# ZhishuaiGuo/DistributedAUC

Hardware: AMD Instinct MI355X
Metric: CoDA train imgs/sec + exact-AUC pos×neg pairs/sec at 1/2/4/8 MI355X (higher is better)
Workload: dtype bf16

## Files before the change

distributedauc_amd/_lib.py:

```python
from __future__ import annotations

import contextlib
import ctypes
import os
import re
from pathlib import Path

PKG_DIR = Path(__file__).resolve().parent
LIB_PATH = Path(os.environ.get("DAUC_LIB", PKG_DIR / "libdauc.so"))
HEADER = PKG_DIR.parent / "include" / "dauc.h"

DAUC_OK = 0
DAUC_EINVAL = -100000
LABEL_I8, LABEL_I32, LABEL_I64 = 1, 2, 3
DTYPE_F32, DTYPE_BF16 = 1, 2
MODE_REFERENCE, MODE_PAPER = 0, 1


class DaucError(RuntimeError):
    """A libdauc.so call returned a non-zero status."""


class GradSeg(ctypes.Structure):

    _fields_ = [("grad", ctypes.c_void_p), ("offset", ctypes.c_int64), ("numel", ctypes.c_int64)]


_vp = ctypes.c_void_p
_i64 = ctypes.c_int64
_int = ctypes.c_int
_f32 = ctypes.c_float
_sz = ctypes.c_size_t

SIGNATURES = {
    "dauc_version": (_int, []),
    "dauc_strerror": (ctypes.c_char_p, [_int]),
    "dauc_label_map_phat": (_int, [_vp, _i64, _i64, _vp, _vp, _vp, _vp, _vp]),
    "dauc_surrogate_workspace_size": (_sz, [_i64]),
    "dauc_surrogate_fwdbwd": (_int, [_vp, _i64, _vp, _int, _i64, _vp, _vp, _vp, _i64, _vp, _vp, _vp,
                                     _vp, _sz, _vp]),
    "dauc_class_sums": (_int, [_vp, _i64, _vp, _int, _i64, _vp, _int, _vp, _sz, _vp]),
    "dauc_surrogate_status": (_int, [_vp, _sz, _vp, _int, _vp]),
    "dauc_alpha_from_sums": (_int, [_vp, _vp, _vp]),
    "dauc_surrogate_logits_fwdbwd": (_int, [_vp, _int, _i64, _vp, _int, _i64, _vp, _vp, _vp, _i64, _vp, _vp,
                                            _vp, _vp, _vp, _sz, _vp]),
    "dauc_class_sums_logits": (_int, [_vp, _int, _i64, _vp, _int, _i64, _vp, _vp, _int, _vp, _sz, _vp]),
    "dauc_pd_update": (_int, [_vp, _vp, _vp, ctypes.POINTER(GradSeg), _int, _vp, _vp, _vp, _f32, _f32,
                              _int, _vp]),
    "dauc_pd_update_dense": (_int, [_vp, _vp, _vp, _vp, _i64, _f32, _f32, _vp]),
    "dauc_coda_finalize": (_int, [_vp, _i64, _int, _vp, _vp, _vp]),
    "dauc_scale_div": (_int, [_vp, _i64, _f32, _vp]),
    "dauc_split_workspace_size": (_sz, [_i64]),
    "dauc_split_scores": (_int, [_vp, _vp, _int, _i64, _vp, _vp, _vp, _vp, _sz, _vp]),
    "dauc_pair_count": (_int, [_vp, _i64, _vp, _i64, _vp, _vp]),
    "dauc_sort_workspace_size": (_sz, [_i64]),
    "dauc_auc_counts_sorted": (_int, [_vp, _i64, _vp, _i64, _vp, _vp, _sz, _vp]),
    "dauc_auc_counts_sorted_labeled": (_int, [_vp, _i64, _vp, _vp, _int, _i64, _i64, _vp, _vp, _vp, _sz, _vp]),
    "dauc_compact_workspace_size": (_sz, [_i64]),
    "dauc_auc_eval_workspace_size": (_sz, [_i64]),
    "dauc_auc_eval_enqueue": (_int, [_vp, _vp, _int, _i64, _int, _int, _vp, _vp, _sz, _vp]),
    "dauc_auc_eval_counts": (_int, [_vp, _vp, _int, _i64, _vp, _vp, _vp, _sz, _vp]),
    "dauc_auc_eval_counts_part": (_int, [_vp, _vp, _int, _i64, _int, _int, _vp, _vp, _vp, _vp, _sz, _vp]),
    "dauc_auc_slot_bytes": (_sz, [_i64, _int]),
    "dauc_auc_eval_compact_part": (_int, [_vp, _vp, _int, _i64, _int, _int, _vp, _vp, _sz, _vp]),
    "dauc_auc_eval_query_part": (_int, [_vp, _vp, _int, _i64, _int, _int, _vp, _vp, _vp, _sz, _vp]),
    "dauc_auc_eval_query_part_sorted": (_int, [_vp, _vp, _int, _i64, _int, _int, _vp, _i64, _vp, _vp, _sz, _vp]),
    "dauc_compact_positives": (_int, [_vp, _vp, _int, _i64, _vp, _vp, _vp, _sz, _vp]),
    "dauc_sort_keys": (_int, [_vp, _i64, _vp, _vp, _sz, _vp]),
    "dauc_bn_workspace_size": (_sz, [_i64, _int]),
    "dauc_bn_act_forward": (_int, [_vp, _int, _i64, _int, _vp, _int, _vp, _vp, _vp, _vp, _f32, _f32, _vp, _vp, _vp,
                                   _vp, _vp, _sz, _vp]),
    "dauc_bn_act_backward": (_int, [_vp, _vp, _vp, _vp, _int, _i64, _int, _int, _vp, _vp, _vp, _vp, _vp, _vp, _vp,
                                    _vp, _sz, _vp]),
    "dauc_maxpool2d_forward": (_int, [_vp, _int, _i64, _int, _int, _int, _int, _int, _int, _vp, _vp, _int, _int,
                                      _vp]),
    "dauc_slab_sum": (_int, [_vp, _i64, _i64, _vp, _vp]),
    "dauc_conv3x3_wgrad_workspace_size": (_sz, [_i64, _int, _int, _int, _int]),
    "dauc_conv3x3_wgrad": (_int, [_vp, _vp, _int, _i64, _int, _int, _int, _int, _int, _int, _int, _vp, _vp, _sz,
                                  _vp]),
    "dauc_maxpool2d_backward": (_int, [_vp, _vp, _int, _i64, _int, _int, _int, _int, _int, _int, _int, _int, _vp,
                                       _vp]),
    "dauc_conv7x7s2_stem_forward": (_int, [_vp, _vp, _int, _i64, _int, _int, _int, _int, _vp, _vp]),
    "dauc_conv7x7s2_stem_wgrad_workspace_size": (_sz, [_i64, _int, _int]),
    "dauc_conv7x7s2_stem_wgrad": (_int, [_vp, _vp, _int, _i64, _int, _int, _int, _int, _vp, _vp, _sz, _vp]),
    "dauc_strided_pick": (_int, [_vp, _int, _i64, _int, _int, _int, _int, _vp, _vp]),
    "dauc_strided_add": (_int, [_vp, _int, _i64, _int, _int, _int, _int, _vp, _vp]),
    "dauc_broadcast_hw": (_int, [_vp, _int, _i64, _i64, _int, _vp, _vp]),
}

TUNING_SIGNATURES = {
    "dauc_surrogate_fwdbwd_variant": (_int, [_vp, _i64, _vp, _int, _i64, _vp, _vp, _vp, _i64, _vp, _vp, _vp,
                                             _vp, _sz, _int, _vp]),
    "dauc_pd_update_dense_variant": (_int, [_vp, _vp, _vp, _vp, _i64, _f32, _f32, _int, _vp]),
    "dauc_pair_count_variant": (_int, [_vp, _i64, _vp, _i64, _vp, _int, _vp]),
    "dauc_set_search_mode": (_int, [_int]),
    "dauc_set_direct_fault": (_int, [_int]),
    "dauc_set_index_form": (_int, [_int]),
    "dauc_probe_tr16": (_int, [_vp, _vp]),
    "dauc_set_wgrad_form": (_int, [_int]),
    "dauc_bn_launch_plan": (_int, [_i64, _int, _int, ctypes.POINTER(_i64)]),
    "dauc_conv3x3_wgrad_launch_plan": (_int, [_i64, _int, _int, _int, _int, _int, _int, _int, ctypes.POINTER(_i64)]),
}
BN_PLAN_WORDS = 12
WGRAD_PLAN_WORDS = 18
TUNING_LIB_PATH = Path(os.environ.get("DAUC_TUNING_LIB", PKG_DIR.parent / "tuning" / "libdauc_tuning.so"))

_lib = None
_tuning = None


@contextlib.contextmanager
def using(lib: ctypes.CDLL):
    global _lib
    prev = load()
    _lib = lib
    try:
        yield lib
    finally:
        _lib = prev


def header_functions(header: Path = HEADER) -> list[str]:
    text = re.sub(r"/\*.*?\*/", "", header.read_text(), flags=re.S)
    return sorted(set(re.findall(r"\b(dauc_[a-z0-9_]+)\s*\(", text)) - {"dauc_grad_seg"})


def load() -> ctypes.CDLL:
    global _lib
    if _lib is not None:
        return _lib
    if not LIB_PATH.exists():
        raise ImportError(
            f"{LIB_PATH} not found: the HIP library must be built first "
            "(python -c 'import __graft_entry__ as g; g.build()' or python distributedauc_amd/build.py). "
            "distributedauc_amd has no CPU fallback."
        )
    _lib = _attach(ctypes.CDLL(str(LIB_PATH)))
    return _lib


def _attach(lib: ctypes.CDLL) -> ctypes.CDLL:
    for name, (res, args) in SIGNATURES.items():
        fn = getattr(lib, name)
        fn.restype = res
        fn.argtypes = args
    for name, (res, args) in TUNING_SIGNATURES.items():
        if hasattr(lib, name):
            fn = getattr(lib, name)
            fn.restype = res
            fn.argtypes = args
    return lib


def tuning() -> ctypes.CDLL:
    global _tuning
    lib = load()
    if all(hasattr(lib, n) for n in TUNING_SIGNATURES):
        return lib
    if _tuning is None:
        if not TUNING_LIB_PATH.exists():
            raise ImportError(f"{TUNING_LIB_PATH} not found: build it with python distributedauc_amd/build.py")
        _tuning = _attach(ctypes.CDLL(str(TUNING_LIB_PATH)))
    return _tuning


def strerror(rc: int) -> str:
    return load().dauc_strerror(rc).decode()


def check(rc: int, what: str) -> None:
    if rc != DAUC_OK:
        raise DaucError(f"{what} failed: {strerror(rc)} (status {rc})")
```

distributedauc_amd/backbone.py:

```python
from __future__ import annotations

import weakref

import torch
import torch.nn as nn
import torch.nn.functional as F

__all__ = [
    "ResNet", "resnet18", "resnet34", "resnet50", "resnet101", "resnet152", "resnext50_32x4d",
    "resnext101_32x8d", "wide_resnet50_2", "wide_resnet101_2", "build_backbone",
]


def _bn_act(fused: bool, bn: nn.BatchNorm2d, x: torch.Tensor, relu: bool = True,
            residual: torch.Tensor | None = None) -> torch.Tensor:
    if fused and bn.training:
        from .fused_bn import bn_act

        return bn_act(x, bn, relu, residual)
    y = bn(x)
    if residual is not None:
        y = y + residual
    return F.relu(y, inplace=True) if relu else y


_shadow_live: list = []


class WeightShadow:

    def __init__(self, model: nn.Module, dgrad_fwd: bool = False, wgrad_hip: bool = False):
        flat = getattr(model, "_dauc_flat", None)
        if flat is None:
            raise RuntimeError("the weight shadow mirrors the FlatState buffer: build CoDA / FlatState first")
        self.src = flat.params
        self._model = weakref.ref(model)
        self.wgrad_hip = bool(wgrad_hip)
        dev = self.src.device
        convs = {id(m.weight): m for m in model.modules() if isinstance(m, nn.Conv2d)}
        idx, foff, vspec, fspec = [], 0, {}, {}
        for _, p, off, _n in flat.entries:
            m = convs.get(id(p))
            if m is None:
                continue
            vspec[id(p)] = (p.shape, p.stride(), off)
            if dgrad_fwd and _dgrad_as_fwd_ok(m):
                co, ci, k, _ = p.shape
                s0, s1, s2, s3 = p.stride()
                r = torch.arange(k)
                src = (off + torch.arange(co).view(1, co, 1, 1) * s0 + torch.arange(ci).view(ci, 1, 1, 1) * s1
                       + (k - 1 - r).view(1, 1, k, 1) * s2 + (k - 1 - r).view(1, 1, 1, k) * s3)
                idx.append(src.permute(0, 2, 3, 1).reshape(-1))
                fspec[id(p)] = ((ci, co, k, k), (k * k * co, 1, k * co, co), foff)
                foff += p.numel()
        self.fidx = torch.cat(idx).to(device=dev, dtype=torch.int32) if idx else None
        self._sets = []
        for _ in range(2):
            buf = torch.empty(self.src.numel(), dtype=torch.bfloat16, device=dev)
            fbuf = torch.empty(foff, dtype=torch.bfloat16, device=dev) if foff else None
            views = {k: torch.as_strided(buf, sh, st, o) for k, (sh, st, o) in vspec.items()}
            flips = {k: torch.as_strided(fbuf, sh, st, o) for k, (sh, st, o) in fspec.items()}
            self._sets.append((buf, fbuf, views, flips))
        self._cur = 1
        self.buf, self.fbuf, self.views, self.flips = self._sets[0]

    def refresh(self, flips: bool = True) -> None:
        m = self._model()
        flat = getattr(m, "_dauc_flat", None) if m is not None else None
        if flat is None or flat.params is not self.src:
            raise RuntimeError("weight shadow is stale: the model's parameters moved to a new FlatState; call "
                               "model.set_weight_shadow(...) again after building it (CoDA does)")
        self._cur ^= 1
        self.buf, self.fbuf, self.views, self.flips = self._sets[self._cur]
        self.buf.copy_(self.src)
        if flips and self.fbuf is not None:
            torch.index_select(self.buf, 0, self.fidx, out=self.fbuf)

    def weight(self, p: torch.Tensor) -> torch.Tensor | None:
        return self.views.get(id(p))

    def flipped(self, p: torch.Tensor) -> torch.Tensor | None:
        return self.flips.get(id(p))


def _dgrad_as_fwd_ok(m: nn.Conv2d) -> bool:
    k = m.kernel_size
    return (k[0] == k[1] and k[0] % 2 == 1 and k[0] > 1 and m.stride == (1, 1) and m.dilation == (1, 1)
            and m.groups == 1 and not isinstance(m.padding, str) and tuple(m.padding) == (k[0] // 2, k[0] // 2)
            and m.padding_mode == "zeros")


def shadow_weight(p: torch.Tensor, dtype: torch.dtype) -> torch.Tensor | None:
    if not _shadow_live or dtype != torch.bfloat16:
        return None
    return _shadow_live[-1].weight(p)


class _ShadowConv(torch.autograd.Function):

    @staticmethod
    def forward(ctx, x, weight, wb, wf, stride, padding, dilation, groups, wgrad_hip=False):
        ctx.stem = False
        if wgrad_hip:
            from . import ops

            ctx.stem = ops.stem_conv_supported(x, wb, stride, padding, dilation, groups)
        if ctx.stem:
            y = ops.stem_conv_forward(x, wb)
        else:
            with torch.autocast("cuda", enabled=False):
                y = F.conv2d(x, wb, None, stride, padding, dilation, groups)
        ctx.save_for_backward(x, wb, wf)
        ctx.conf = (list(stride), list(padding), list(dilation), groups)
        ctx.wgrad_hip = bool(wgrad_hip)
        return y

    @staticmethod
    def backward(ctx, gy):
        x, wb, wf = ctx.saved_tensors
        stride, padding, dilation, groups = ctx.conf
        nx, nw = bool(ctx.needs_input_grad[0]), bool(ctx.needs_input_grad[1])
        dx = dw = None
        if nw and ctx.stem and gy.dtype == torch.bfloat16:
            from . import ops

            dw = ops.stem_conv_wgrad(x, gy.contiguous(memory_format=torch.channels_last))
        elif nw and ctx.wgrad_hip and wb.shape[2:] == (3, 3):
            from . import ops

            gyc = gy.contiguous(memory_format=torch.channels_last)
            if ops.conv3x3_wgrad_supported(x, gyc, stride, padding, dilation, groups):
                dw = ops.conv3x3_wgrad(x, gyc, stride[0])
        mw = nw and dw is None
        if wf is not None and nx:
            dx = F.conv2d(gy.contiguous(memory_format=torch.channels_last), wf, None, 1, padding, 1, 1)
            if mw:
                dw = torch.ops.aten.convolution_backward(gy, x, wb, None, stride, padding, dilation, False, [0, 0],
                                                         groups, [False, True, False])[1].float()
        elif nx or mw:
            dx, dwb, _ = torch.ops.aten.convolution_backward(gy, x, wb, None, stride, padding, dilation, False,
                                                              [0, 0], groups, [nx, mw, False])
            if mw:
                dw = dwb.float()
        return dx, dw, None, None, None, None, None, None, None


def _cw(conv: nn.Conv2d, x: torch.Tensor) -> torch.Tensor:
    wb = shadow_weight(conv.weight, torch.bfloat16) if x.is_cuda else None
    if (wb is None or conv.bias is not None or conv.padding_mode != "zeros" or isinstance(conv.padding, str)
            or not torch.is_autocast_enabled("cuda")):
        return conv(x)
    if x.dtype == torch.float32:
        x = x.to(torch.bfloat16)
    if x.dtype != torch.bfloat16:
        return conv(x)
    sh = _shadow_live[-1]
    wf = sh.flipped(conv.weight) if torch.is_grad_enabled() else None
    return _ShadowConv.apply(x, conv.weight, wb, wf, conv.stride, conv.padding, conv.dilation, conv.groups,
                             sh.wgrad_hip)


class _GlobalAvgPoolCL(torch.autograd.Function):

    @staticmethod
    def forward(ctx, x):
        ctx.shape = x.shape
        return F.adaptive_avg_pool2d(x, 1)

    @staticmethod
    def backward(ctx, g):
        N, C, H, W = ctx.shape
        gs = g / (H * W)
        if gs.is_cuda and gs.dtype == torch.bfloat16 and C % 8 == 0:
            from . import ops

            return ops.broadcast_hw(gs, H, W)
        out = torch.empty((N, C, H, W), dtype=gs.dtype, device=gs.device, memory_format=torch.channels_last)
        out.copy_(gs.expand(N, C, H, W))
        return out


def _global_pool(pool: nn.Module, x: torch.Tensor) -> torch.Tensor:
    if (x.is_cuda and x.dim() == 4 and x.is_contiguous(memory_format=torch.channels_last)
            and isinstance(pool, nn.AdaptiveAvgPool2d) and pool.output_size in (1, (1, 1)) and torch.is_grad_enabled()):
        return _GlobalAvgPoolCL.apply(x)
    return pool(x)


def _c1(gemm: bool, conv: nn.Conv2d, x: torch.Tensor) -> torch.Tensor:
    if gemm:
        from .conv1x1 import conv1x1

        return conv1x1(conv, x)
    return conv(x)


def _conv(cin: int, cout: int, k: int, stride: int = 1, groups: int = 1) -> nn.Conv2d:
    return nn.Conv2d(cin, cout, kernel_size=k, stride=stride, padding=k // 2, groups=groups, bias=False)


class BasicBlock(nn.Module):
    expansion = 1

    def __init__(self, cin, planes, stride=1, downsample=None, groups=1, base_width=64):
        super().__init__()
        if groups != 1 or base_width != 64:
            raise ValueError("BasicBlock supports groups=1, base_width=64 only")
        self.conv1 = _conv(cin, planes, 3, stride)
        self.bn1 = nn.BatchNorm2d(planes)
        self.conv2 = _conv(planes, planes, 3)
        self.bn2 = nn.BatchNorm2d(planes)
        self.relu = nn.ReLU(inplace=True)
        self.downsample = downsample
        self.fused_bn = False
        self.gemm_conv1x1 = False

    def forward(self, x):
        f = self.fused_bn
        skip = x if self.downsample is None else _bn_act(f, self.downsample[1], _c1(self.gemm_conv1x1,
                                                                                  self.downsample[0], x),
                                                         relu=False)
        y = _bn_act(f, self.bn1, _cw(self.conv1, x))
        return _bn_act(f, self.bn2, _cw(self.conv2, y), residual=skip)


class Bottleneck(nn.Module):

    expansion = 4

    def __init__(self, cin, planes, stride=1, downsample=None, groups=1, base_width=64):
        super().__init__()
        width = int(planes * (base_width / 64.0)) * groups
        self.conv1 = _conv(cin, width, 1)
        self.bn1 = nn.BatchNorm2d(width)
        self.conv2 = _conv(width, width, 3, stride, groups)
        self.bn2 = nn.BatchNorm2d(width)
        self.conv3 = _conv(width, planes * self.expansion, 1)
        self.bn3 = nn.BatchNorm2d(planes * self.expansion)
        self.relu = nn.ReLU(inplace=True)
        self.downsample = downsample
        self.fused_bn = False
        self.gemm_conv1x1 = False

    def forward(self, x):
        f, g = self.fused_bn, self.gemm_conv1x1
        down = None if self.downsample is None else self.downsample[0]
        if g and x.is_cuda:
            from .conv1x1 import conv1x1_skip

            h, skip = conv1x1_skip(self.conv1, x, down, skip_grad_owned=f and self.training)
        else:
            h, skip = _c1(g, self.conv1, x), (x if down is None else _c1(g, down, x))
        if down is not None:
            skip = _bn_act(f, self.downsample[1], skip, relu=False)
        y = _bn_act(f, self.bn1, h)
        y = _bn_act(f, self.bn2, _cw(self.conv2, y))
        return _bn_act(f, self.bn3, _c1(g, self.conv3, y), residual=skip)


class ResNet(nn.Module):

    def __init__(self, block, layers, num_classes: int = 2, groups: int = 1, width_per_group: int = 64,
                 zero_init_residual: bool = False, head: str = "softmax"):
        super().__init__()
        if head not in ("softmax", "logits"):
            raise ValueError("head must be 'softmax' or 'logits'")
        self.groups = groups
        self.base_width = width_per_group
        self.inplanes = 64
        self.conv1 = nn.Conv2d(3, 64, kernel_size=7, stride=2, padding=3, bias=False)
        self.bn1 = nn.BatchNorm2d(64)
        self.relu = nn.ReLU(inplace=True)
        self.maxpool = nn.MaxPool2d(kernel_size=3, stride=2, padding=1)
        self.layer1 = self._stage(block, 64, layers[0], 1)
        self.layer2 = self._stage(block, 128, layers[1], 2)
        self.layer3 = self._stage(block, 256, layers[2], 2)
        self.layer4 = self._stage(block, 512, layers[3], 2)
        self.avgpool = nn.AdaptiveAvgPool2d((1, 1))
        self.fc = nn.Linear(512 * block.expansion, num_classes)
        self.softmax = nn.Softmax(dim=1) if head == "softmax" else nn.Identity()
        for m in self.modules():
            if isinstance(m, nn.Conv2d):
                nn.init.kaiming_normal_(m.weight, mode="fan_out", nonlinearity="relu")
            elif isinstance(m, nn.BatchNorm2d):
                nn.init.ones_(m.weight)
                nn.init.zeros_(m.bias)
        if zero_init_residual:
            for m in self.modules():
                if isinstance(m, Bottleneck):
                    nn.init.zeros_(m.bn3.weight)
                elif isinstance(m, BasicBlock):
                    nn.init.zeros_(m.bn2.weight)

    def _stage(self, block, planes, blocks, stride):
        down = None
        cout = planes * block.expansion
        if stride != 1 or self.inplanes != cout:
            down = nn.Sequential(_conv(self.inplanes, cout, 1, stride), nn.BatchNorm2d(cout))
        mods = [block(self.inplanes, planes, stride, down, self.groups, self.base_width)]
        self.inplanes = cout
        mods += [block(cout, planes, 1, None, self.groups, self.base_width) for _ in range(1, blocks)]
        return nn.Sequential(*mods)

    fused_bn = False
    _counted_bns: list = []
    _wshadow: WeightShadow | None = None

    def set_weight_shadow(self, enabled: bool = True, dgrad_fwd: bool = True, wgrad_hip: bool = True) -> "ResNet":
        self._wshadow = WeightShadow(self, dgrad_fwd=dgrad_fwd, wgrad_hip=wgrad_hip) if enabled else None
        return self

    def set_fused_bn(self, enabled: bool = True) -> "ResNet":
        self.fused_bn = bool(enabled)
        self._counted_bns = []
        for m in self.modules():
            if isinstance(m, (BasicBlock, Bottleneck)):
                m.fused_bn = self.fused_bn
            if isinstance(m, nn.BatchNorm2d):
                batched = self.fused_bn and m.track_running_stats and m.momentum is not None
                m._dauc_counted = batched
                if batched:
                    self._counted_bns.append(m)
        return self

    def set_gemm_conv1x1(self, enabled: bool = True) -> "ResNet":
        for m in self.modules():
            if isinstance(m, (BasicBlock, Bottleneck)):
                m.gemm_conv1x1 = bool(enabled)
        return self

    def features(self, x):
        if self.fused_bn and self.training and x.is_cuda and self._counted_bns:
            torch._foreach_add_([m.num_batches_tracked for m in self._counted_bns], 1)
        live = (self._wshadow is not None and x.is_cuda and torch.is_autocast_enabled("cuda")
                and torch.get_autocast_dtype("cuda") == torch.bfloat16)
        if live:
            self._wshadow.refresh(flips=torch.is_grad_enabled())
            _shadow_live.append(self._wshadow)
        try:
            x = _bn_act(self.fused_bn, self.bn1, _cw(self.conv1, x))
            if self.fused_bn and x.is_cuda:
                from .pool import max_pool2d

                x = max_pool2d(x, self.maxpool)
            else:
                x = self.maxpool(x)
            x = self.layer4(self.layer3(self.layer2(self.layer1(x))))
        finally:
            if live:
                _shadow_live.pop()
        return torch.flatten(_global_pool(self.avgpool, x), 1)

    def forward(self, x):
        return self.softmax(self.fc(self.features(x)))


_SPECS = {
    "resnet18": (BasicBlock, [2, 2, 2, 2], {}),
    "resnet34": (BasicBlock, [3, 4, 6, 3], {}),
    "resnet50": (Bottleneck, [3, 4, 6, 3], {}),
    "resnet101": (Bottleneck, [3, 4, 23, 3], {}),
    "resnet152": (Bottleneck, [3, 8, 36, 3], {}),
    "resnext50_32x4d": (Bottleneck, [3, 4, 6, 3], {"groups": 32, "width_per_group": 4}),
    "resnext101_32x8d": (Bottleneck, [3, 4, 23, 3], {"groups": 32, "width_per_group": 8}),
    "wide_resnet50_2": (Bottleneck, [3, 4, 6, 3], {"width_per_group": 128}),
    "wide_resnet101_2": (Bottleneck, [3, 4, 23, 3], {"width_per_group": 128}),
}


def build_backbone(arch: str, pretrained: bool | str = False, **kwargs) -> ResNet:
    block, layers, extra = _SPECS[arch]
    model = ResNet(block, layers, **{**extra, **kwargs})
    if pretrained:
        if pretrained is True:
            raise RuntimeError("pretrained weights need a local state_dict path (no network in this build)")
        sd = torch.load(pretrained, map_location="cpu", weights_only=True)
        sd = {k: v for k, v in sd.items() if not k.startswith("fc.")}
        model.load_state_dict(sd, strict=False)
    return model


def _factory(name):
    def make(pretrained=False, progress=True, **kwargs):
        return build_backbone(name, pretrained, **kwargs)

    make.__name__ = name
    make.__doc__ = f"{name} with a 2-way softmax head (resnet.py factory of the same name)."
    return make


resnet18 = _factory("resnet18")
resnet34 = _factory("resnet34")
resnet50 = _factory("resnet50")
resnet101 = _factory("resnet101")
resnet152 = _factory("resnet152")
resnext50_32x4d = _factory("resnext50_32x4d")
resnext101_32x8d = _factory("resnext101_32x8d")
wide_resnet50_2 = _factory("wide_resnet50_2")
wide_resnet101_2 = _factory("wide_resnet101_2")
```

distributedauc_amd/conv1x1.py:

```python
from __future__ import annotations

import contextlib
import os

import torch
import torch.nn as nn
import torch.nn.functional as F

from . import _lib
from .ops import _ptr, _stream, check, strided_add_, strided_pick

__all__ = ["conv1x1", "conv1x1_skip", "Conv1x1Function", "Conv1x1SkipFunction", "plans", "dump_plans"]

plans: dict = {}

_DOWNSAMPLE_BWD = os.environ.get("DAUC_DOWNSAMPLE_BWD", "gemm")
PLANS_FILE = os.environ.get("DAUC_CONV1X1_PLANS", os.path.join(os.path.dirname(__file__), "conv1x1_plans.json"))


def _plan_key(key) -> str:
    M, cin, cout, dtype, direction = key
    return f"{M},{cin},{cout},{str(dtype).replace('torch.', '')},{direction}"


def _arch() -> str:
    return torch.cuda.get_device_properties(torch.cuda.current_device()).gcnArchName.split(":")[0]


def _load_plans() -> None:
    if not PLANS_FILE or not os.path.exists(PLANS_FILE):
        return
    import json

    dtypes = {"bfloat16": torch.bfloat16, "float16": torch.float16, "float32": torch.float32}
    with open(PLANS_FILE) as f:
        doc = json.load(f)
    if doc.get("arch") and torch.cuda.is_available() and doc["arch"] != _arch():
        return
    for k, eng in doc.get("plans", {}).items():
        M, cin, cout, dt, direction = k.split(",")
        plans.setdefault((int(M), int(cin), int(cout), dtypes[dt], direction), eng)


def dump_plans(path: str) -> None:
    import json

    with open(path, "w") as f:
        json.dump({"device": torch.cuda.get_device_name(0) if torch.cuda.is_available() else None,
                   "arch": _arch() if torch.cuda.is_available() else None,
                   "plans": {_plan_key(k): v for k, v in sorted(plans.items(), key=lambda kv: _plan_key(kv[0]))}},
                  f, indent=1)



def _timed(fn, reps=3):
    torch.cuda.synchronize()
    best = float("inf")
    for _ in range(reps):
        a, b = torch.cuda.Event(enable_timing=True), torch.cuda.Event(enable_timing=True)
        a.record()
        fn()
        b.record()
        b.synchronize()
        best = min(best, a.elapsed_time(b))
    return best


_FORCE = os.environ.get("DAUC_CONV1X1", "auto")
_loaded: list = []
_fixed: list = []


@contextlib.contextmanager
def fixed_engine(name: str = "gemm"):
    _fixed.append(name)
    try:
        yield
    finally:
        _fixed.pop()


def _choose(key, candidates: dict):
    if _fixed:
        eng = next((n for n in candidates if n.startswith(_fixed[-1])), None)
        if eng == "gemm8" and "gemm32" in candidates:
            eng = "gemm32"
        if eng is not None:
            return eng
    if not _loaded:
        _load_plans()
        _loaded.append(True)
    eng = plans.get(key) if _FORCE == "auto" else None
    if eng is None and _FORCE != "auto":
        eng = next((n for n in candidates if n.startswith(_FORCE)), None)
        if eng == "gemm8" and "gemm32" in candidates:
            eng = "gemm32"
        if eng is not None:
            plans[key] = eng
    if eng is None:
        times = {name: _timed(fn) for name, fn in candidates.items()}
        eng = min(times, key=times.get)
        plans[key] = eng
    return eng


def _wgrad_gemm(g2, x2, slabs):
    M, cout = g2.shape
    cin = x2.shape[1]
    if slabs == 1:
        return torch.mm(g2.t(), x2, out_dtype=torch.float32)
    part = torch.bmm(g2.view(slabs, M // slabs, cout).transpose(1, 2), x2.view(slabs, M // slabs, cin),
                     out_dtype=torch.float32)
    if (cout * cin) % 4:
        return part.sum(0)
    out = torch.empty((cout, cin), dtype=torch.float32, device=part.device)
    check(_lib.load().dauc_slab_sum(_ptr(part), slabs, cout * cin, _ptr(out), _stream(part.device)),
          "dauc_slab_sum")
    return out


def _low(weight, dtype):
    from .backbone import shadow_weight

    wb = shadow_weight(weight, dtype)
    return wb.detach() if wb is not None else weight.detach().to(dtype)


def _fwd(x, weight):
    N, cin, H, W = x.shape
    cout = weight.shape[0]
    M = N * H * W
    wc = _low(weight, x.dtype).reshape(cout, cin)
    x2 = x.permute(0, 2, 3, 1).reshape(M, cin)
    with torch.autocast("cuda", enabled=False):
        key = (M, cin, cout, x.dtype, "fwd")
        eng = _choose(key, {"gemm": lambda: torch.mm(x2, wc.t()),
                            "conv": lambda: F.conv2d(x, wc.view(cout, cin, 1, 1))})
        if eng == "gemm":
            y = torch.mm(x2, wc.t()).view(N, H, W, cout).permute(0, 3, 1, 2)
        else:
            y = F.conv2d(x, wc.view(cout, cin, 1, 1)).contiguous(memory_format=torch.channels_last)
    return y, wc


def _prep_grad(gy, x, cout):
    N, cin, H, W = x.shape
    gy = gy.to(x.dtype).contiguous(memory_format=torch.channels_last)
    return gy, gy.permute(0, 2, 3, 1).reshape(N * H * W, cout)


def _conv_dgrad(gy, x, wc):
    cout, cin = wc.shape
    return torch.ops.aten.convolution_backward(gy, x, wc.view(cout, cin, 1, 1), None, [1, 1], [0, 0], [1, 1],
                                               False, [0, 0], 1, [True, False, False])[0]


def _fconv_dgrad(gy, wc):
    cout, cin = wc.shape
    return F.conv2d(gy, wc.t().contiguous().view(cin, cout, 1, 1)).contiguous(memory_format=torch.channels_last)


def _dgrad(gy, g2, x, wc):
    N, cin, H, W = x.shape
    cout = wc.shape[0]
    M = N * H * W
    with torch.autocast("cuda", enabled=False):
        eng = _choose((M, cin, cout, x.dtype, "dgrad"),
                      {"gemm": lambda: torch.mm(g2, wc), "conv": lambda: _conv_dgrad(gy, x, wc),
                       "fconv": lambda: _fconv_dgrad(gy, wc)})
        if eng == "gemm":
            return torch.mm(g2, wc).view(N, H, W, cin).permute(0, 3, 1, 2)
        if eng == "fconv":
            return _fconv_dgrad(gy, wc)
        return _conv_dgrad(gy, x, wc).contiguous(memory_format=torch.channels_last)


def _dgrad_acc(base, gy, g2, x, wc):
    N, cin, H, W = x.shape
    cout = wc.shape[0]
    M = N * H * W
    b2 = base.permute(0, 2, 3, 1).reshape(M, cin)
    with torch.autocast("cuda", enabled=False):
        key = (M, cin, cout, x.dtype, "dgrad_acc")
        if not _loaded:
            _load_plans()
            _loaded.append(True)
        eng = None if _fixed else plans.get(key)
        if eng is None and _fixed:
            eng = _choose(key, {"gemm": None, "conv": None, "fconv": None})
        elif eng is None:
            scratch = base.clone(memory_format=torch.channels_last)
            s2 = scratch.permute(0, 2, 3, 1).reshape(M, cin)
            eng = _choose(key, {"gemm": lambda: s2.addmm_(g2, wc),
                                "conv": lambda: scratch.add_(_conv_dgrad(gy, x, wc)),
                                "fconv": lambda: scratch.add_(_fconv_dgrad(gy, wc))})
            del scratch, s2
        if eng == "gemm":
            b2.addmm_(g2, wc)
        elif eng == "fconv":
            base.add_(_fconv_dgrad(gy, wc))
        else:
            base.add_(_conv_dgrad(gy, x, wc))
    return base


def _wgrad(gy, g2, x, wc, wdtype):
    N, cin, H, W = x.shape
    cout = wc.shape[0]
    M = N * H * W
    x2 = x.permute(0, 2, 3, 1).reshape(M, cin)
    with torch.autocast("cuda", enabled=False):
        def conv_w():
            return torch.ops.aten.convolution_backward(gy, x, wc.view(cout, cin, 1, 1), None, [1, 1], [0, 0], [1, 1],
                                                       False, [0, 0], 1, [False, True, False])[1]

        cands = {"conv": conv_w}
        for s in (8, 32, 128):
            if M % s == 0 and M // s >= 64:
                cands[f"gemm{s}"] = (lambda s=s: _wgrad_gemm(g2, x2, s))
        eng = _choose((M, cin, cout, x.dtype, "wgrad"), cands)
        if eng == "conv":
            dw = conv_w().reshape(cout, cin).to(wdtype)
        else:
            dw = _wgrad_gemm(g2, x2, int(eng[4:])).to(wdtype)
    return dw.view(cout, cin, 1, 1)


def _cl_ok(t: torch.Tensor) -> bool:
    return (t.is_cuda and t.dtype == torch.bfloat16 and t.dim() == 4 and t.shape[1] % 8 == 0
            and t.is_contiguous(memory_format=torch.channels_last) and t.data_ptr() % 16 == 0)


def _pick(x: torch.Tensor, s: int) -> torch.Tensor:
    if _cl_ok(x):
        return strided_pick(x, s)
    return x[:, :, ::s, ::s].contiguous(memory_format=torch.channels_last)


def _add_strided(dx: torch.Tensor, src: torch.Tensor, s: int) -> None:
    if _cl_ok(dx) and _cl_ok(src):
        strided_add_(dx, src, s)
    else:
        dx[:, :, ::s, ::s].add_(src)


class Conv1x1Function(torch.autograd.Function):
    @staticmethod
    def forward(ctx, x, weight):
        y, wc = _fwd(x, weight)
        ctx.save_for_backward(x, wc)
        ctx.wdtype = weight.dtype
        return y

    @staticmethod
    def backward(ctx, gy):
        x, wc = ctx.saved_tensors
        gy, g2 = _prep_grad(gy, x, wc.shape[0])
        dx = _dgrad(gy, g2, x, wc) if ctx.needs_input_grad[0] else None
        dw = _wgrad(gy, g2, x, wc, ctx.wdtype) if ctx.needs_input_grad[1] else None
        return dx, dw


class Conv1x1SkipFunction(torch.autograd.Function):

    @staticmethod
    def forward(ctx, x, w1, wd, skip_grad_owned, down_stride=1):
        y1, wc1 = _fwd(x, w1)
        ctx.down_stride = int(down_stride)
        if wd is None:
            skip, wcd = x, None
        elif down_stride == 1:
            skip, wcd = _fwd(x, wd)
        else:
            wcd = _low(wd, x.dtype).reshape(wd.shape[0], wd.shape[1])
            with torch.autocast("cuda", enabled=False):
                skip = F.conv2d(x, wcd.view(*wd.shape), stride=down_stride).contiguous(
                    memory_format=torch.channels_last)
        ctx.save_for_backward(x, wc1, wcd)
        ctx.wdtypes = (w1.dtype, None if wd is None else wd.dtype)
        ctx.skip_grad_owned = bool(skip_grad_owned)
        return y1, skip

    @staticmethod
    def backward(ctx, g1, gs):
        x, wc1, wcd = ctx.saved_tensors
        dx = dw1 = dwd = None
        gy1 = g21 = gyd = g2d = None
        if g1 is not None:
            gy1, g21 = _prep_grad(g1, x, wc1.shape[0])
        strided = wcd is not None and ctx.down_stride != 1
        s = ctx.down_stride
        xd = x
        dx_down = dwd_s = None
        if gs is not None and strided and _DOWNSAMPLE_BWD == "miopen":
            gsd = gs.to(x.dtype).contiguous(memory_format=torch.channels_last)
            cout, cin = wcd.shape
            with torch.autocast("cuda", enabled=False):
                dx_down, dwd_s, _ = torch.ops.aten.convolution_backward(
                    gsd, x, wcd.view(cout, cin, 1, 1), None, [s, s], [0, 0], [1, 1], False, [0, 0], 1,
                    [bool(ctx.needs_input_grad[0]), bool(ctx.needs_input_grad[2]), False])
        elif gs is not None and wcd is not None:
            if strided:
                xd = _pick(x, s)
            gyd, g2d = _prep_grad(gs, xd, wcd.shape[0])
        if ctx.needs_input_grad[0]:
            if gs is None:
                base = None
            elif wcd is None:
                base = gs.to(x.dtype).contiguous(memory_format=torch.channels_last)
                if base is gs and not ctx.skip_grad_owned:
                    base = base.clone(memory_format=torch.channels_last)
            elif strided:
                base = None if dx_down is None else dx_down.contiguous(memory_format=torch.channels_last)
            else:
                base = _dgrad(gyd, g2d, x, wcd)
            if g1 is None:
                dx = base
            elif base is None:
                dx = _dgrad(gy1, g21, x, wc1)
            else:
                dx = _dgrad_acc(base, gy1, g21, x, wc1)
            if strided and gs is not None and dx_down is None:
                if dx is None:
                    dx = torch.zeros_like(x, memory_format=torch.channels_last)
                _add_strided(dx, _dgrad(gyd, g2d, xd, wcd), s)
        if ctx.needs_input_grad[1] and g1 is not None:
            dw1 = _wgrad(gy1, g21, x, wc1, ctx.wdtypes[0])
        if wcd is not None and ctx.needs_input_grad[2] and gs is not None:
            if dwd_s is not None:
                dwd = dwd_s.to(ctx.wdtypes[1]).view(wcd.shape[0], wcd.shape[1], 1, 1)
            else:
                dwd = _wgrad(gyd, g2d, xd, wcd, ctx.wdtypes[1])
        return dx, dw1, dwd, None, None


def conv1x1(conv: nn.Conv2d, x: torch.Tensor) -> torch.Tensor:
    if (conv.kernel_size != (1, 1) or conv.stride != (1, 1) or conv.groups != 1 or conv.bias is not None
            or conv.padding != (0, 0) or x.device.type != "cuda"
            or not x.is_contiguous(memory_format=torch.channels_last)):
        return conv(x)
    if torch.is_autocast_enabled("cuda") and x.dtype == torch.float32:
        x = x.to(torch.get_autocast_dtype("cuda"))
    return Conv1x1Function.apply(x, conv.weight)


def _gemm_ok(conv: nn.Conv2d | None, x: torch.Tensor, any_stride: bool = False) -> bool:
    return conv is None or (conv.kernel_size == (1, 1) and conv.groups == 1 and conv.bias is None
                            and conv.padding == (0, 0) and conv.dilation == (1, 1)
                            and (conv.stride == (1, 1) or (any_stride and conv.stride[0] == conv.stride[1])))


def conv1x1_skip(conv: nn.Conv2d, x: torch.Tensor, down: nn.Conv2d | None = None, skip_grad_owned: bool = False):
    if (x.device.type != "cuda" or not x.is_contiguous(memory_format=torch.channels_last)
            or not _gemm_ok(conv, x) or not _gemm_ok(down, x, any_stride=True)):
        return conv1x1(conv, x), (x if down is None else conv1x1(down, x))
    if torch.is_autocast_enabled("cuda") and x.dtype == torch.float32:
        x = x.to(torch.get_autocast_dtype("cuda"))
    return Conv1x1SkipFunction.apply(x, conv.weight, None if down is None else down.weight, skip_grad_owned,
                                     1 if down is None else down.stride[0])
```

distributedauc_amd/csrc/bn_act.hip:

```cpp

#include <hip/hip_bf16.h>

#include <initializer_list>
#include <type_traits>

#include "dauc_internal.h"
#ifdef DAUC_TUNING
#include "dauc_tuning.h"
#endif

namespace dauc {
namespace {

constexpr int kBnThreads = 256;
constexpr int kDefaultPartThreads = 512;
constexpr int kMaxRowBlocks = 2048;
constexpr int kFinThreads = 1024;
constexpr int kFinSubsets = kFinThreads / 16;

constexpr int kRowBlockTarget = 256;
static_assert(kRowBlockTarget >= 1 && kRowBlockTarget <= kMaxRowBlocks, "partial rows fit the workspace");
constexpr int kUnroll = 8;
constexpr int kFwdUnroll = kUnroll;
constexpr int kBwdUnroll = kUnroll / 2;
constexpr int kFinUnroll = 4;
constexpr int kApplyVecs = 4;
constexpr int64_t kApplyBlockVecs = int64_t(kApplyVecs) * kBnThreads;

template <typename T>
struct VecT;
template <>
struct VecT<__hip_bfloat16> {
    static constexpr int N = 8;
};
template <>
struct VecT<float> {
    static constexpr int N = 4;
};

template <typename T>
using RawT = typename std::conditional<sizeof(T) == 2, uint4, f32x4>::type;

template <typename T>
__device__ __forceinline__ RawT<T> load_raw(const T* p) {
    return *reinterpret_cast<const RawT<T>*>(p);
}

__device__ __forceinline__ void cvt(const uint4& u, float (&v)[8]) {
    const unsigned w[4] = {u.x, u.y, u.z, u.w};
#pragma unroll
    for (int i = 0; i < 4; ++i) {
        v[2 * i] = __uint_as_float(w[i] << 16);
        v[2 * i + 1] = __uint_as_float(w[i] & 0xffff0000u);
    }
}

__device__ __forceinline__ void cvt(const f32x4& u, float (&v)[4]) {
#pragma unroll
    for (int i = 0; i < 4; ++i) v[i] = u[i];
}

template <typename T, int N>
__device__ __forceinline__ void load_vec(const T* p, float (&v)[N]) {
    cvt(load_raw(p), v);
}

__device__ __forceinline__ unsigned bf16_bits(float f) {
    const unsigned b = __float_as_uint(f);
    if ((b & 0x7fffffffu) > 0x7f800000u) return (b >> 16) | 0x40u;
    return (b + 0x7fffu + ((b >> 16) & 1u)) >> 16;
}

__device__ __forceinline__ void store_vec(__hip_bfloat16* p, const float (&v)[8]) {
    uint4 u;
    u.x = bf16_bits(v[0]) | (bf16_bits(v[1]) << 16);
    u.y = bf16_bits(v[2]) | (bf16_bits(v[3]) << 16);
    u.z = bf16_bits(v[4]) | (bf16_bits(v[5]) << 16);
    u.w = bf16_bits(v[6]) | (bf16_bits(v[7]) << 16);
    *reinterpret_cast<uint4*>(p) = u;
}

__device__ __forceinline__ void store_vec(float* p, const float (&v)[4]) {
    f32x4 u;
#pragma unroll
    for (int i = 0; i < 4; ++i) u[i] = v[i];
    *reinterpret_cast<f32x4*>(p) = u;
}

__device__ __forceinline__ unsigned store_vec_mask(__hip_bfloat16* p, const float (&v)[8]) {
    unsigned b[8], m = 0u;
#pragma unroll
    for (int i = 0; i < 8; ++i) {
        b[i] = bf16_bits(v[i]);
        m |= unsigned(b[i] - 1u < 0x7f80u) << i;
    }
    uint4 u;
    u.x = b[0] | (b[1] << 16);
    u.y = b[2] | (b[3] << 16);
    u.z = b[4] | (b[5] << 16);
    u.w = b[6] | (b[7] << 16);
    *reinterpret_cast<uint4*>(p) = u;
    return m;
}

__device__ __forceinline__ unsigned store_vec_mask(float* p, const float (&v)[4]) {
    unsigned m = 0u;
#pragma unroll
    for (int i = 0; i < 4; ++i) m |= unsigned(__float_as_uint(v[i]) - 1u < 0x7f800000u) << i;
    store_vec(p, v);
    return m;
}

struct Geometry {
    int N;
    int CT;
    int TPR;
    int RPB;
    int ctiles;
    int nrb;
    int64_t rows;
};

int make_geometry(int64_t M, int C, int elem_bytes, Geometry& g, int threads = kBnThreads) {
    g.N = 16 / elem_bytes;
    if (M <= 0 || C <= 0 || C % g.N != 0) return DAUC_EINVAL;
    const int CV = C / g.N;
    g.TPR = CV <= kBnThreads ? CV : kBnThreads;
    if (kBnThreads % g.TPR != 0 || CV % g.TPR != 0) return DAUC_EINVAL;
    g.CT = g.TPR * g.N;
    g.ctiles = C / g.CT;
    g.RPB = threads / g.TPR;
    int64_t target = (kRowBlockTarget + g.ctiles - 1) / g.ctiles;
    const int64_t passes = (M + g.RPB - 1) / g.RPB;
    if (target > passes) target = passes;
    if (target < 1) target = 1;
    int64_t rows = (M + target - 1) / target;
    rows = (rows + g.RPB - 1) / g.RPB * g.RPB;
    g.rows = rows;
    g.nrb = static_cast<int>((M + rows - 1) / rows);
    return DAUC_OK;
}

template <typename T, bool STATS, bool RELU, int TH, bool MASK = false>
__global__ __launch_bounds__(TH) void bn_partial_kernel(
    const T* __restrict__ x, const T* __restrict__ dy, const T* __restrict__ y, T* __restrict__ dz, int64_t M,
    int C, int CT, int64_t rows_per_block, const float* __restrict__ center, float* __restrict__ partials,
    const unsigned char* __restrict__ mask) {
    constexpr int N = VecT<T>::N;
    __shared__ float red[2 * TH * N];
    const int TPR = CT / N;
    const int RPB = TH / TPR;
    const int cl = (threadIdx.x % TPR) * N;
    const int c0 = blockIdx.y * CT + cl;
    const int r0 = threadIdx.x / TPR;
    const int64_t rs = int64_t(blockIdx.x) * rows_per_block;
    const int64_t re = (rs + rows_per_block < M) ? rs + rows_per_block : M;
    constexpr int NP = STATS ? 3 : 2;

    float k[N], s1[N], s2[N];
    if (STATS) load_vec(x + rs * C + c0, k);
#pragma unroll
    for (int i = 0; i < N; ++i) {
        if (!STATS) k[i] = center[c0 + i];
        s1[i] = 0.f;
        s2[i] = 0.f;
    }
    auto visit = [&](int64_t r) {
        const int64_t off = r * C + c0;
        float xv[N];
        load_vec(x + off, xv);
        if (STATS) {
#pragma unroll
            for (int i = 0; i < N; ++i) {
                const float d = xv[i] - k[i];
                s1[i] += d;
                s2[i] += d * d;
            }
        } else {
            float gv[N];
            load_vec(dy + off, gv);
            if (RELU && MASK) {
                const unsigned m = mask[off / N];
#pragma unroll
                for (int i = 0; i < N; ++i) gv[i] = (m >> i) & 1u ? gv[i] : 0.f;
            } else if (RELU) {
                float yv[N];
                load_vec(y + off, yv);
#pragma unroll
                for (int i = 0; i < N; ++i) gv[i] = yv[i] > 0.f ? gv[i] : 0.f;
            }
            if (dz) store_vec(dz + off, gv);
#pragma unroll
            for (int i = 0; i < N; ++i) {
                s1[i] += gv[i];
                s2[i] += gv[i] * (xv[i] - k[i]);
            }
        }
    };
    constexpr int U = STATS ? kFwdUnroll : kBwdUnroll;
    int64_t r = rs + r0;
    const int64_t step = int64_t(RPB) * U;
    for (; r + step - RPB < re; r += step) {
        RawT<T> xr[U], gr[U], yr[U];
        unsigned mr[U];
#pragma unroll
        for (int u = 0; u < U; ++u) {
            const int64_t off = (r + int64_t(u) * RPB) * C + c0;
            xr[u] = load_raw(x + off);
            if (!STATS) gr[u] = load_raw(dy + off);
            if (!STATS && RELU && MASK) mr[u] = mask[off / N];
            else if (!STATS && RELU) yr[u] = load_raw(y + off);
        }
#pragma unroll
        for (int u = 0; u < U; ++u) {
            float xv[N];
            cvt(xr[u], xv);
            if (STATS) {
#pragma unroll
                for (int i = 0; i < N; ++i) {
                    const float d = xv[i] - k[i];
                    s1[i] += d;
                    s2[i] += d * d;
                }
            } else {
                float gv[N];
                cvt(gr[u], gv);
                if (RELU && MASK) {
#pragma unroll
                    for (int i = 0; i < N; ++i) gv[i] = (mr[u] >> i) & 1u ? gv[i] : 0.f;
                } else if (RELU) {
                    float yv[N];
                    cvt(yr[u], yv);
#pragma unroll
                    for (int i = 0; i < N; ++i) gv[i] = yv[i] > 0.f ? gv[i] : 0.f;
                }
                if (dz) store_vec(dz + (r + int64_t(u) * RPB) * C + c0, gv);
#pragma unroll
                for (int i = 0; i < N; ++i) {
                    s1[i] += gv[i];
                    s2[i] += gv[i] * (xv[i] - k[i]);
                }
            }
        }
    }
    for (; r < re; r += RPB) visit(r);

    float* r1 = red;
    float* r2 = red + TH * N;
#pragma unroll
    for (int i = 0; i < N; ++i) {
        r1[r0 * CT + cl + i] = s1[i];
        r2[r0 * CT + cl + i] = s2[i];
    }
    __syncthreads();
    for (int j = threadIdx.x; j < 2 * CT; j += TH) {
        const int stat = j / CT, c = j % CT;
        const float* src = stat ? r2 : r1;
        float acc = 0.f;
        for (int q = 0; q < RPB; ++q) acc += src[q * CT + c];
        partials[(int64_t(blockIdx.x) * NP + stat) * C + blockIdx.y * CT + c] = acc;
    }
    if (STATS && r0 == 0) {
#pragma unroll
        for (int i = 0; i < N; ++i) partials[(int64_t(blockIdx.x) * NP + 2) * C + c0 + i] = k[i];
    }
}

template <bool STATS>
__device__ __forceinline__ void sum_partials(const float* __restrict__ partials, int nrb, int64_t M, int64_t rows,
                                             int C, int cbase, double (*red)[kFinSubsets][64], double& t1,
                                             double& t2) {
    constexpr int NP = STATS ? 3 : 2;
    constexpr int FU = kFinUnroll;
    const int cq = threadIdx.x % 16, j = threadIdx.x / 16;
    const int c = cbase + cq * 4;
    double a1[4] = {0, 0, 0, 0}, a2[4] = {0, 0, 0, 0};
    auto fold = [&](int rb, const f32x4& p1, const f32x4& p2, const f32x4& pk) {
        if (STATS) {
            const int64_t r0 = int64_t(rb) * rows;
            const double nb = double((M - r0) < rows ? (M - r0) : rows);
#pragma unroll
            for (int i = 0; i < 4; ++i) {
                const double k = pk[i], s1 = p1[i];
                a1[i] += s1 + nb * k;
                a2[i] += double(p2[i]) + 2.0 * k * s1 + nb * k * k;
            }
        } else {
#pragma unroll
            for (int i = 0; i < 4; ++i) {
                a1[i] += p1[i];
                a2[i] += p2[i];
            }
        }
    };
    auto ld = [&](int rb, int q) {
        return *reinterpret_cast<const f32x4*>(partials + (int64_t(rb) * NP + q) * C + c);
    };
    if (c < C) {
        int rb = j;
        for (; rb + (FU - 1) * kFinSubsets < nrb; rb += FU * kFinSubsets) {
            f32x4 p1[FU], p2[FU], pk[FU];
#pragma unroll
            for (int u = 0; u < FU; ++u) {
                p1[u] = ld(rb + u * kFinSubsets, 0);
                p2[u] = ld(rb + u * kFinSubsets, 1);
                if (STATS) pk[u] = ld(rb + u * kFinSubsets, 2);
            }
#pragma unroll
            for (int u = 0; u < FU; ++u) fold(rb + u * kFinSubsets, p1[u], p2[u], pk[u]);
        }
        for (; rb < nrb; rb += kFinSubsets) {
            const f32x4 p1 = ld(rb, 0), p2 = ld(rb, 1);
            f32x4 pk;
            if (STATS) pk = ld(rb, 2);
            fold(rb, p1, p2, pk);
        }
    }
#pragma unroll
    for (int i = 0; i < 4; ++i) {
        red[0][j][cq * 4 + i] = a1[i];
        red[1][j][cq * 4 + i] = a2[i];
    }
    __syncthreads();
#pragma unroll
    for (int s = kFinSubsets / 2; s >= 1; s >>= 1) {
        if (j < s) {
#pragma unroll
            for (int i = 0; i < 4; ++i) {
                red[0][j][cq * 4 + i] += red[0][j + s][cq * 4 + i];
                red[1][j][cq * 4 + i] += red[1][j + s][cq * 4 + i];
            }
        }
        __syncthreads();
    }
    t1 = 0.0;
    t2 = 0.0;
    if (threadIdx.x < 64) {
        t1 = red[0][0][threadIdx.x];
        t2 = red[1][0][threadIdx.x];
    }
}

__global__ __launch_bounds__(kFinThreads) void bn_fwd_finalize_kernel(
    const float* __restrict__ partials, int nrb, int64_t rows, int64_t M, int C, const float* __restrict__ gamma,
    const float* __restrict__ beta, float* __restrict__ running_mean, float* __restrict__ running_var,
    float momentum, float eps, float* __restrict__ save_mean, float* __restrict__ save_invstd,
    float* __restrict__ scale, float* __restrict__ beta_out, float* __restrict__ mean_out) {
    __shared__ double red[2][kFinSubsets][64];
    double sx, sxx;
    sum_partials<true>(partials, nrb, M, rows, C, blockIdx.x * 64, red, sx, sxx);
    const int c = blockIdx.x * 64 + threadIdx.x;
    if (threadIdx.x >= 64 || c >= C) return;
    const double mean = sx / double(M);
    double var = sxx / double(M) - mean * mean;
    if (var < 0.0) var = 0.0;
    const double invstd = 1.0 / sqrt(var + double(eps));
    save_mean[c] = static_cast<float>(mean);
    save_invstd[c] = static_cast<float>(invstd);
    const double g = gamma ? gamma[c] : 1.0, b = beta ? beta[c] : 0.0;
    scale[c] = static_cast<float>(g * invstd);
    beta_out[c] = static_cast<float>(b);
    mean_out[c] = static_cast<float>(mean);
    if (running_mean) {
        const double unbiased = M > 1 ? var * double(M) / double(M - 1) : var;
        running_mean[c] = static_cast<float>((1.0 - momentum) * running_mean[c] + momentum * mean);
        running_var[c] = static_cast<float>((1.0 - momentum) * running_var[c] + momentum * unbiased);
    }
}

__global__ __launch_bounds__(kFinThreads) void bn_bwd_finalize_kernel(
    const float* __restrict__ partials, int nrb, int64_t M, int C, const float* __restrict__ gamma,
    const float* __restrict__ save_mean, const float* __restrict__ save_invstd, float* __restrict__ dgamma,
    float* __restrict__ dbeta, float* __restrict__ ca, float* __restrict__ cb, float* __restrict__ cc,
    float* __restrict__ cm) {
    __shared__ double red[2][kFinSubsets][64];
    double sg, sgx;
    sum_partials<false>(partials, nrb, M, 0, C, blockIdx.x * 64, red, sg, sgx);
    const int c = blockIdx.x * 64 + threadIdx.x;
    if (threadIdx.x >= 64 || c >= C) return;
    const double inv = save_invstd[c], mean = save_mean[c];
    const double g = gamma ? gamma[c] : 1.0;
    if (dgamma) dgamma[c] = static_cast<float>(sgx * inv);
    if (dbeta) dbeta[c] = static_cast<float>(sg);
    const double a = g * inv;
    const double b = -g * inv * inv * inv * sgx / double(M);
    ca[c] = static_cast<float>(a);
    cb[c] = static_cast<float>(b);
    cc[c] = static_cast<float>(-a * sg / double(M));
    cm[c] = save_mean[c];
}

template <typename T, bool BWD, int GMODE, bool RELU, bool RES, bool HOIST, bool MASK = false>
__global__ __launch_bounds__(kBnThreads) void bn_elementwise_kernel(
    const T* __restrict__ x, const T* __restrict__ g_in, const T* __restrict__ aux, T* __restrict__ out,
    int64_t nvec, int CV, const float* __restrict__ p0, const float* __restrict__ p1, const float* __restrict__ p2,
    const float* __restrict__ p3, unsigned char* __restrict__ mask) {
    constexpr int N = VecT<T>::N;
    auto body = [&](int64_t v, const float* P0, const float* P1, const float* P2, const float* P3) {
        const int64_t off = v * N;
        float xv[N];
        load_vec(x + off, xv);
        float o[N];
        if (!BWD) {
            float rv[N];
            if (RES) load_vec(aux + off, rv);
#pragma unroll
            for (int i = 0; i < N; ++i) {
                float t = (xv[i] - P3[i]) * P0[i] + P1[i];
                if (RES) t += rv[i];
                o[i] = (RELU && t < 0.f) ? 0.f : t;
            }
        } else {
            float gv[N];
            load_vec(g_in + off, gv);
            if (GMODE == 1 && MASK) {
                const unsigned m = mask[v];
#pragma unroll
                for (int i = 0; i < N; ++i) gv[i] = (m >> i) & 1u ? gv[i] : 0.f;
            } else if (GMODE == 1) {
                float yv[N];
                load_vec(aux + off, yv);
#pragma unroll
                for (int i = 0; i < N; ++i) gv[i] = yv[i] > 0.f ? gv[i] : 0.f;
            }
#pragma unroll
            for (int i = 0; i < N; ++i) o[i] = P0[i] * gv[i] + P1[i] * (xv[i] - P3[i]) + P2[i];
        }
        if constexpr (!BWD && RELU && MASK)
            mask[v] = static_cast<unsigned char>(store_vec_mask(out + off, o));
        else
            store_vec(out + off, o);
    };
    auto params = [&](int cv, float (&q0)[N], float (&q1)[N], float (&q2)[N], float (&q3)[N]) {
#pragma unroll
        for (int i = 0; i < N; ++i) {
            q0[i] = p0[cv * N + i];
            q1[i] = p1[cv * N + i];
            q2[i] = BWD ? p2[cv * N + i] : 0.f;
            q3[i] = p3[cv * N + i];
        }
    };
    const int64_t base = int64_t(blockIdx.x) * kApplyVecs * kBnThreads + threadIdx.x;
    float q0[N], q1[N], q2[N], q3[N];
    if (HOIST) params(threadIdx.x % CV, q0, q1, q2, q3);
    if (int64_t(blockIdx.x + 1) * kApplyVecs * kBnThreads <= nvec) {
#pragma unroll
        for (int u = 0; u < kApplyVecs; ++u) {
            const int64_t v = base + int64_t(u) * kBnThreads;
            if (!HOIST) params(static_cast<int>(v % CV), q0, q1, q2, q3);
            body(v, q0, q1, q2, q3);
        }
    } else {
        for (int u = 0; u < kApplyVecs; ++u) {
            const int64_t v = base + int64_t(u) * kBnThreads;
            if (v >= nvec) break;
            if (!HOIST) params(static_cast<int>(v % CV), q0, q1, q2, q3);
            body(v, q0, q1, q2, q3);
        }
    }
}

struct BnWs {
    float* partials;
    float* c0;
    float* c1;
    float* c2;
    float* c3;
};

size_t ws_bytes_for(int C) {
    return (size_t(kMaxRowBlocks) * 3 + 4) * size_t(C) * sizeof(float) + 256;
}

BnWs carve(void* ws, int C) {
    char* p = static_cast<char*>(ws);
    BnWs w;
    w.partials = reinterpret_cast<float*>(p);
    w.c0 = w.partials + size_t(kMaxRowBlocks) * 3 * C;
    w.c1 = w.c0 + C;
    w.c2 = w.c1 + C;
    w.c3 = w.c2 + C;
    return w;
}

bool aligned16p(const void* p) { return (reinterpret_cast<uintptr_t>(p) & 15u) == 0; }

int64_t apply_blocks(int64_t nvec) { return (nvec + kApplyBlockVecs - 1) / kApplyBlockVecs; }
bool apply_hoists(int CV) { return kBnThreads % CV == 0; }

template <typename T, bool BWD, int GMODE, bool RELU, bool RES, bool MASK = false>
int launch_elementwise(const T* x, const T* g_in, const T* aux, T* out, int64_t M, int C, const float* p0,
                       const float* p1, const float* p2, const float* p3, hipStream_t st,
                       unsigned char* mask = nullptr) {
    constexpr int N = VecT<T>::N;
    const int CV = C / N;
    const int64_t nvec = M * CV;
    const int64_t grid = apply_blocks(nvec);
    if (grid > 0x7fffffffLL) return DAUC_EINVAL;
    if (apply_hoists(CV))
        hipLaunchKernelGGL((bn_elementwise_kernel<T, BWD, GMODE, RELU, RES, true, MASK>), dim3(unsigned(grid)),
                           dim3(kBnThreads), 0, st, x, g_in, aux, out, nvec, CV, p0, p1, p2, p3, mask);
    else
        hipLaunchKernelGGL((bn_elementwise_kernel<T, BWD, GMODE, RELU, RES, false, MASK>), dim3(unsigned(grid)),
                           dim3(kBnThreads), 0, st, x, g_in, aux, out, nvec, CV, p0, p1, p2, p3, mask);
    return launch_status();
}

template <typename T, bool STATS, bool RELU, bool MASK = false>
void launch_partial(int th, const Geometry& g, const T* x, const T* dy, const T* y, T* dz, int64_t M, int C,
                    const float* center, float* partials, hipStream_t st, const unsigned char* mask = nullptr) {
    const dim3 grid(g.nrb, g.ctiles);
    if (th == 1024)
        hipLaunchKernelGGL((bn_partial_kernel<T, STATS, RELU, 1024, MASK>), grid, dim3(1024), 0, st, x, dy, y, dz, M,
                           C, g.CT, g.rows, center, partials, mask);
    else if (th == 512)
        hipLaunchKernelGGL((bn_partial_kernel<T, STATS, RELU, 512, MASK>), grid, dim3(512), 0, st, x, dy, y, dz, M,
                           C, g.CT, g.rows, center, partials, mask);
    else
        hipLaunchKernelGGL((bn_partial_kernel<T, STATS, RELU, 256, MASK>), grid, dim3(256), 0, st, x, dy, y, dz, M,
                           C, g.CT, g.rows, center, partials, mask);
}

template <typename T>
int bn_forward_t(const T* x, int64_t M, int C, const T* res, int relu, const float* gamma, const float* beta,
                 float* running_mean, float* running_var, float momentum, float eps, T* y, unsigned char* mask,
                 float* save_mean, float* save_invstd, void* ws, size_t ws_bytes, hipStream_t st) {
    Geometry g;
    const int th = kDefaultPartThreads;
    if (make_geometry(M, C, sizeof(T), g, th) != DAUC_OK) return DAUC_EINVAL;
    if (ws == nullptr || ws_bytes < ws_bytes_for(C) || !aligned16p(ws)) return DAUC_EINVAL;
    if ((running_mean == nullptr) != (running_var == nullptr)) return DAUC_EINVAL;
    const BnWs w = carve(ws, C);
    launch_partial<T, true, false>(th, g, x, nullptr, nullptr, nullptr, M, C, nullptr, w.partials, st);
    hipLaunchKernelGGL(bn_fwd_finalize_kernel, dim3((C + 63) / 64), dim3(kFinThreads), 0, st, w.partials, g.nrb,
                       g.rows, M, C, gamma, beta, running_mean, running_var, momentum, eps, save_mean, save_invstd, w.c0, w.c1, w.c3);
    int rc = launch_status();
    if (rc != DAUC_OK) return rc;
    if (relu && mask && res)
        return launch_elementwise<T, false, 0, true, true, true>(x, nullptr, res, y, M, C, w.c0, w.c1, nullptr, w.c3, st,
                                                                mask);
    if (relu && mask)
        return launch_elementwise<T, false, 0, true, false, true>(x, nullptr, nullptr, y, M, C, w.c0, w.c1, nullptr,
                                                                 w.c3, st, mask);
    if (relu && res)
        return launch_elementwise<T, false, 0, true, true>(x, nullptr, res, y, M, C, w.c0, w.c1, nullptr, w.c3, st);
    if (relu) return launch_elementwise<T, false, 0, true, false>(x, nullptr, nullptr, y, M, C, w.c0, w.c1, nullptr, w.c3, st);
    if (res) return launch_elementwise<T, false, 0, false, true>(x, nullptr, res, y, M, C, w.c0, w.c1, nullptr, w.c3, st);
    return launch_elementwise<T, false, 0, false, false>(x, nullptr, nullptr, y, M, C, w.c0, w.c1, nullptr, w.c3, st);
}

template <typename T>
int bn_backward_t(const T* dy, const T* y, const unsigned char* mask, const T* x, int64_t M, int C, int relu,
                  const float* gamma, const float* save_mean, const float* save_invstd, T* dres, T* dx, float* dgamma,
                  float* dbeta, void* ws, size_t ws_bytes, hipStream_t st) {
    Geometry g;
    const int th = kDefaultPartThreads;
    if (make_geometry(M, C, sizeof(T), g, th) != DAUC_OK) return DAUC_EINVAL;
    if (ws == nullptr || ws_bytes < ws_bytes_for(C) || !aligned16p(ws)) return DAUC_EINVAL;
    if (relu && y == nullptr && mask == nullptr) return DAUC_EINVAL;
    const BnWs w = carve(ws, C);
    if (relu && mask)
        launch_partial<T, false, true, true>(th, g, x, dy, nullptr, dres, M, C, save_mean, w.partials, st, mask);
    else if (relu)
        launch_partial<T, false, true>(th, g, x, dy, y, dres, M, C, save_mean, w.partials, st);
    else
        launch_partial<T, false, false>(th, g, x, dy, nullptr, dres, M, C, save_mean, w.partials, st);
    hipLaunchKernelGGL(bn_bwd_finalize_kernel, dim3((C + 63) / 64), dim3(kFinThreads), 0, st, w.partials, g.nrb, M, C,
                       gamma, save_mean, save_invstd, dgamma, dbeta, w.c0, w.c1, w.c2, w.c3);
    int rc = launch_status();
    if (rc != DAUC_OK) return rc;
    if (dres)
        return launch_elementwise<T, true, 2, false, false>(x, dres, nullptr, dx, M, C, w.c0, w.c1, w.c2, w.c3, st);
    if (relu && mask)
        return launch_elementwise<T, true, 1, false, false, true>(x, dy, nullptr, dx, M, C, w.c0, w.c1, w.c2, w.c3, st,
                                                                 const_cast<unsigned char*>(mask));
    if (relu) return launch_elementwise<T, true, 1, false, false>(x, dy, y, dx, M, C, w.c0, w.c1, w.c2, w.c3, st);
    return launch_elementwise<T, true, 0, false, false>(x, dy, nullptr, dx, M, C, w.c0, w.c1, w.c2, w.c3, st);
}

bool all_aligned(std::initializer_list<const void*> ps) {
    for (const void* p : ps)
        if (p != nullptr && !aligned16p(p)) return false;
    return true;
}

}
}

using namespace dauc;

extern "C" {

size_t dauc_bn_workspace_size(int64_t M, int C) {
    (void)M;
    return C > 0 ? ws_bytes_for(C) : 0;
}

int dauc_bn_act_forward(const void* x, int dtype, int64_t M, int C, const void* residual, int relu,
                        const float* gamma, const float* beta, float* running_mean, float* running_var,
                        float momentum, float eps, void* y, uint8_t* relu_mask, float* save_mean, float* save_invstd,
                        void* workspace, size_t workspace_bytes, dauc_stream_t stream) {
    if (x == nullptr || y == nullptr || save_mean == nullptr || save_invstd == nullptr) return DAUC_EINVAL;
    if (!all_aligned({x, residual, y})) return DAUC_EINVAL;
    if (relu_mask != nullptr && !relu) return DAUC_EINVAL;
    hipStream_t st = as_hip(stream);
    if (dtype == DAUC_DTYPE_BF16)
        return bn_forward_t(static_cast<const __hip_bfloat16*>(x), M, C, static_cast<const __hip_bfloat16*>(residual),
                            relu, gamma, beta, running_mean, running_var, momentum, eps,
                            static_cast<__hip_bfloat16*>(y), relu_mask, save_mean, save_invstd, workspace,
                            workspace_bytes, st);
    if (dtype == DAUC_DTYPE_F32)
        return bn_forward_t(static_cast<const float*>(x), M, C, static_cast<const float*>(residual), relu, gamma,
                            beta, running_mean, running_var, momentum, eps, static_cast<float*>(y), relu_mask,
                            save_mean, save_invstd, workspace, workspace_bytes, st);
    return DAUC_EINVAL;
}

int dauc_bn_act_backward(const void* dy, const void* y, const uint8_t* relu_mask, const void* x, int dtype, int64_t M,
                         int C, int relu, const float* gamma, const float* save_mean, const float* save_invstd,
                         void* dres, void* dx, float* dgamma, float* dbeta, void* workspace, size_t workspace_bytes,
                         dauc_stream_t stream) {
    if (dy == nullptr || x == nullptr || dx == nullptr || save_mean == nullptr || save_invstd == nullptr)
        return DAUC_EINVAL;
    if (!all_aligned({dy, y, x, dres, dx})) return DAUC_EINVAL;
    hipStream_t st = as_hip(stream);
    if (dtype == DAUC_DTYPE_BF16)
        return bn_backward_t(static_cast<const __hip_bfloat16*>(dy), static_cast<const __hip_bfloat16*>(y), relu_mask,
                             static_cast<const __hip_bfloat16*>(x), M, C, relu, gamma, save_mean, save_invstd,
                             static_cast<__hip_bfloat16*>(dres), static_cast<__hip_bfloat16*>(dx), dgamma, dbeta,
                             workspace, workspace_bytes, st);
    if (dtype == DAUC_DTYPE_F32)
        return bn_backward_t(static_cast<const float*>(dy), static_cast<const float*>(y), relu_mask,
                             static_cast<const float*>(x), M, C, relu, gamma, save_mean, save_invstd,
                             static_cast<float*>(dres), static_cast<float*>(dx), dgamma, dbeta, workspace,
                             workspace_bytes, st);
    return DAUC_EINVAL;
}

#ifdef DAUC_TUNING
int dauc_bn_launch_plan(int64_t M, int C, int dtype, int64_t out[DAUC_BN_PLAN_WORDS]) {
    if (out == nullptr || (dtype != DAUC_DTYPE_BF16 && dtype != DAUC_DTYPE_F32)) return DAUC_EINVAL;
    Geometry g;
    const int rc = make_geometry(M, C, dtype == DAUC_DTYPE_BF16 ? 2 : 4, g, kDefaultPartThreads);
    if (rc != DAUC_OK) return rc;
    const int CV = C / g.N;
    out[0] = g.TPR;
    out[1] = g.RPB;
    out[2] = g.ctiles;
    out[3] = g.nrb;
    out[4] = g.rows;
    out[5] = int64_t(g.RPB) * kFwdUnroll;
    out[6] = int64_t(g.RPB) * kBwdUnroll;
    out[7] = int64_t(kFinSubsets) * kFinUnroll;
    out[8] = kFinSubsets;
    out[9] = kApplyBlockVecs;
    out[10] = apply_blocks(M * CV);
    out[11] = apply_hoists(CV) ? 1 : 0;
    return DAUC_OK;
}
#endif

}
```

distributedauc_amd/csrc/dauc_internal.h:

```cpp
#pragma once

#include <hip/hip_runtime.h>
#include <stdint.h>

#include "../../include/dauc.h"

namespace dauc {

constexpr int kWave = 64;

typedef float f32x4 __attribute__((ext_vector_type(4)));

inline hipStream_t as_hip(dauc_stream_t s) { return reinterpret_cast<hipStream_t>(s); }

inline int launch_status() {
    hipError_t e = hipGetLastError();
    return e == hipSuccess ? DAUC_OK : -static_cast<int>(e);
}


__device__ __forceinline__ double wave_sum(double v) {
#pragma unroll
    for (int off = 32; off > 0; off >>= 1) v += __shfl_xor(v, off, kWave);
    return v;
}

__device__ __forceinline__ unsigned long long wave_sum(unsigned long long v) {
#pragma unroll
    for (int off = 32; off > 0; off >>= 1) v += __shfl_xor(v, off, kWave);
    return v;
}

template <int K>
__device__ __forceinline__ void block_sum(double (&v)[K], double* scratch) {
    const int lane = threadIdx.x & (kWave - 1);
    const int wid = threadIdx.x / kWave;
    const int nw = blockDim.x / kWave;
#pragma unroll
    for (int k = 0; k < K; ++k) v[k] = wave_sum(v[k]);
    if (lane == 0) {
#pragma unroll
        for (int k = 0; k < K; ++k) scratch[k * nw + wid] = v[k];
    }
    __syncthreads();
#pragma unroll
    for (int k = 0; k < K; ++k) {
        double s = 0.0;
        for (int w = 0; w < nw; ++w) s += scratch[k * nw + w];
        v[k] = s;
    }
    __syncthreads();
}

typedef __attribute__((address_space(1))) unsigned long long gu64;
typedef __attribute__((address_space(1))) unsigned gu32;

__device__ __forceinline__ void store_sc1(double* p, double v) {
    __hip_atomic_store((gu64*)p, static_cast<unsigned long long>(__double_as_longlong(v)), __ATOMIC_RELAXED,
                       __HIP_MEMORY_SCOPE_AGENT);
}

__device__ __forceinline__ double load_sc1(const double* p) {
    return __longlong_as_double(static_cast<long long>(
        __hip_atomic_load((gu64*)p, __ATOMIC_RELAXED, __HIP_MEMORY_SCOPE_AGENT)));
}

__device__ __forceinline__ bool arrive_last(unsigned* counter, unsigned nblocks, int* lds_flag) {
    if (threadIdx.x == 0) {
        asm volatile("s_waitcnt vmcnt(0)" ::: "memory");
        const unsigned t = __hip_atomic_fetch_add((gu32*)counter, 1u, __ATOMIC_RELAXED, __HIP_MEMORY_SCOPE_AGENT);
        const int last = (t == nblocks - 1);
        if (last) __hip_atomic_store((gu32*)counter, 0u, __ATOMIC_RELAXED, __HIP_MEMORY_SCOPE_AGENT);
        *lds_flag = last;
    }
    __syncthreads();
    __builtin_amdgcn_fence(__ATOMIC_ACQUIRE, "wavefront");
    return *lds_flag != 0;
}

inline bool label_dtype_ok(int label_dtype) {
    return label_dtype == DAUC_LABEL_I8 || label_dtype == DAUC_LABEL_I32 || label_dtype == DAUC_LABEL_I64;
}

template <typename F>
int with_labels(const void* labels, int label_dtype, F&& f) {
    switch (label_dtype) {
        case DAUC_LABEL_I8: return f(static_cast<const int8_t*>(labels));
        case DAUC_LABEL_I32: return f(static_cast<const int32_t*>(labels));
        case DAUC_LABEL_I64: return f(static_cast<const int64_t*>(labels));
        default: return DAUC_EINVAL;
    }
}

}
```

distributedauc_amd/fused_bn.py:

```python
from __future__ import annotations

import torch
import torch.nn as nn

from . import _lib
from .ops import _ptr, _stream, check, workspaces

__all__ = ["supported", "bn_act", "BnActFunction"]

_DTYPES = {torch.float32: 1, torch.bfloat16: 2}


def supported(x: torch.Tensor) -> bool:
    if x.dim() != 4 or x.device.type != "cuda" or x.dtype not in _DTYPES:
        return False
    if not x.is_contiguous(memory_format=torch.channels_last) or x.data_ptr() % 16:
        return False
    vec = 16 // x.element_size()
    C = x.shape[1]
    if C % vec:
        return False
    cv = C // vec
    tpr = min(cv, 256)
    return 256 % tpr == 0 and cv % tpr == 0


class BnActFunction(torch.autograd.Function):

    @staticmethod
    def forward(ctx, x, weight, bias, residual, running_mean, running_var, momentum, eps, relu):
        N, C, H, W = x.shape
        M = N * H * W
        dev = x.device
        L = _lib.load()
        y = torch.empty_like(x, memory_format=torch.channels_last)
        mask = torch.empty(M * C * x.element_size() // 16, dtype=torch.uint8, device=dev) if relu else None
        mean = torch.empty(C, dtype=torch.float32, device=dev)
        invstd = torch.empty(C, dtype=torch.float32, device=dev)
        ws = workspaces.get(dev, "bn", L.dauc_bn_workspace_size(M, C))
        if residual is not None:
            if residual.shape != x.shape or residual.dtype != x.dtype:
                raise ValueError("residual must match x in shape and dtype")
            residual = residual.contiguous(memory_format=torch.channels_last)
        check(L.dauc_bn_act_forward(_ptr(x), _DTYPES[x.dtype], M, C, _ptr(residual), int(relu), _ptr(weight),
                                    _ptr(bias), _ptr(running_mean), _ptr(running_var), float(momentum), float(eps),
                                    _ptr(y), _ptr(mask), _ptr(mean), _ptr(invstd), _ptr(ws), ws.numel(), _stream(dev)),
              "dauc_bn_act_forward")
        ctx.save_for_backward(x, mask, weight, mean, invstd)
        ctx.relu = bool(relu)
        ctx.has_residual = residual is not None
        ctx.has_bias = bias is not None
        return y

    @staticmethod
    def backward(ctx, dy):
        x, mask, weight, mean, invstd = ctx.saved_tensors
        N, C, H, W = x.shape
        M = N * H * W
        dev = x.device
        L = _lib.load()
        dy = dy.contiguous(memory_format=torch.channels_last)
        if dy.dtype != x.dtype:
            dy = dy.to(x.dtype)
        dx = torch.empty_like(x, memory_format=torch.channels_last)
        dres = torch.empty_like(x, memory_format=torch.channels_last) if ctx.has_residual else None
        dgamma = torch.empty(C, dtype=torch.float32, device=dev) if weight is not None else None
        dbeta = torch.empty(C, dtype=torch.float32, device=dev) if ctx.has_bias else None
        ws = workspaces.get(dev, "bn", L.dauc_bn_workspace_size(M, C))
        check(L.dauc_bn_act_backward(_ptr(dy), None, _ptr(mask), _ptr(x), _DTYPES[x.dtype], M, C, int(ctx.relu),
                                     _ptr(weight), _ptr(mean), _ptr(invstd), _ptr(dres), _ptr(dx), _ptr(dgamma),
                                     _ptr(dbeta), _ptr(ws), ws.numel(), _stream(dev)),
              "dauc_bn_act_backward")
        return dx, dgamma, dbeta, dres, None, None, None, None, None


def bn_act(x: torch.Tensor, bn: nn.BatchNorm2d, relu: bool = True,
           residual: torch.Tensor | None = None) -> torch.Tensor:
    if x.device.type != "cuda":
        raise RuntimeError("fused BN runs on the GPU only (libdauc.so); no CPU path")
    if not supported(x):
        raise ValueError(f"fused BN needs a channels-last bf16/fp32 tensor with a supported channel count, "
                         f"got {tuple(x.shape)} {x.dtype}")
    momentum = 0.0 if bn.momentum is None else bn.momentum
    rm, rv = (bn.running_mean, bn.running_var) if bn.track_running_stats else (None, None)
    if bn.track_running_stats and bn.num_batches_tracked is not None and not getattr(bn, "_dauc_counted", False):
        bn.num_batches_tracked.add_(1)
        if bn.momentum is None:
            momentum = 1.0 / float(bn.num_batches_tracked.item())
    return BnActFunction.apply(x, bn.weight, bn.bias, residual, rm, rv, momentum, bn.eps, relu)
```

include/dauc.h:

```cpp
#ifndef DAUC_H_
#define DAUC_H_

#include <stddef.h>
#include <stdint.h>

#ifdef __cplusplus
extern "C" {
#endif

typedef struct ihipStream_t* dauc_stream_t;

#define DAUC_OK 0
#define DAUC_EINVAL (-100000)

#define DAUC_LABEL_I8 1
#define DAUC_LABEL_I32 2
#define DAUC_LABEL_I64 3

#define DAUC_DTYPE_F32 1
#define DAUC_DTYPE_BF16 2

#define DAUC_MODE_REFERENCE 0
#define DAUC_MODE_PAPER 1


int dauc_version(void);

const char* dauc_strerror(int status);


int dauc_label_map_phat(const int64_t* labels, int64_t B, int64_t split_index, int8_t* y_out,
                        float* lcounts, const float* gcounts, float* p_hat, dauc_stream_t stream);


size_t dauc_surrogate_workspace_size(int64_t B);

int dauc_surrogate_fwdbwd(const float* h, int64_t h_stride, const void* y, int y_dtype, int64_t B,
                          const float* abalpha, const float* p_hat, float* dh, int64_t dh_stride,
                          double* out64, float* grad3, float* loss, void* workspace,
                          size_t workspace_bytes, dauc_stream_t stream);

int dauc_surrogate_status(void* workspace, size_t workspace_bytes, unsigned* status_out, int clear,
                          dauc_stream_t stream);

int dauc_class_sums(const float* h, int64_t h_stride, const void* y, int y_dtype, int64_t B,
                    double* sums4, int accumulate, void* workspace, size_t workspace_bytes,
                    dauc_stream_t stream);

int dauc_surrogate_logits_fwdbwd(const void* z, int z_dtype, int64_t ldz, const void* y, int y_dtype,
                                 int64_t B, const float* abalpha, const float* p_hat, void* dz, int64_t lddz,
                                 float* h_out, double* out64, float* grad3, float* loss, void* workspace,
                                 size_t workspace_bytes, dauc_stream_t stream);

int dauc_class_sums_logits(const void* z, int z_dtype, int64_t ldz, const void* y, int y_dtype, int64_t B,
                           float* h_out, double* sums4, int accumulate, void* workspace, size_t workspace_bytes,
                           dauc_stream_t stream);

int dauc_alpha_from_sums(const double* sums4, float* alpha, dauc_stream_t stream);


typedef struct dauc_grad_seg {
    const float* grad;
    int64_t offset;
    int64_t numel;
} dauc_grad_seg;

int dauc_pd_update(float* w, const float* w0, float* w_avg, const dauc_grad_seg* segs, int nseg,
                   float* scalars, const float* grad3, const float* anchor3, float lr,
                   float inv_gamma, int mode, dauc_stream_t stream);

int dauc_pd_update_dense(float* w, const float* g, const float* w0, float* w_avg, int64_t n,
                         float lr, float inv_gamma, dauc_stream_t stream);


int dauc_coda_finalize(float* flat, int64_t n_avg, int world, float* lcounts, float* gcounts,
                       dauc_stream_t stream);

int dauc_scale_div(float* x, int64_t n, float divisor, dauc_stream_t stream);


size_t dauc_split_workspace_size(int64_t n);

int dauc_split_scores(const float* scores, const void* labels, int label_dtype, int64_t n,
                      float* pos_out, float* neg_out, int64_t* stats, void* workspace,
                      size_t workspace_bytes, dauc_stream_t stream);

size_t dauc_compact_workspace_size(int64_t n);
int dauc_compact_positives(const float* scores, const void* labels, int label_dtype, int64_t n,
                           float* pos_out, int64_t* stats, void* workspace, size_t workspace_bytes,
                           dauc_stream_t stream);

int dauc_pair_count(const float* pos, int64_t P, const float* neg, int64_t N,
                    unsigned long long* wins_ties, dauc_stream_t stream);

size_t dauc_sort_workspace_size(int64_t n);

int dauc_auc_counts_sorted(const float* pos, int64_t P, const float* neg, int64_t N,
                           unsigned long long* wins_ties, void* workspace, size_t workspace_bytes,
                           dauc_stream_t stream);

int dauc_auc_counts_sorted_labeled(const float* pos, int64_t P, const float* scores, const void* labels,
                                   int label_dtype, int64_t begin, int64_t end, unsigned long long* wins_ties,
                                   unsigned long long* nonfinite, void* workspace, size_t workspace_bytes,
                                   dauc_stream_t stream);

size_t dauc_auc_eval_workspace_size(int64_t n);
int dauc_auc_eval_enqueue(const float* scores, const void* labels, int label_dtype, int64_t n, int part, int parts,
                          int64_t* part_out, void* workspace, size_t workspace_bytes, dauc_stream_t stream);

int dauc_auc_eval_counts(const float* scores, const void* labels, int label_dtype, int64_t n, int64_t* out,
                         int64_t* pinned, void* workspace, size_t workspace_bytes, dauc_stream_t stream);

int dauc_auc_eval_counts_part(const float* scores, const void* labels, int label_dtype, int64_t n, int part,
                              int parts, int64_t* out, int64_t* part_counts, int64_t* pinned, void* workspace,
                              size_t workspace_bytes, dauc_stream_t stream);

size_t dauc_auc_slot_bytes(int64_t n, int parts);
int dauc_auc_eval_compact_part(const float* scores, const void* labels, int label_dtype, int64_t n, int part,
                               int parts, void* slot, void* workspace, size_t workspace_bytes, dauc_stream_t stream);
int dauc_auc_eval_query_part(const float* scores, const void* labels, int label_dtype, int64_t n, int part, int parts,
                             const void* slots, int64_t* part_out, void* workspace, size_t workspace_bytes,
                             dauc_stream_t stream);
int dauc_auc_eval_query_part_sorted(const float* scores, const void* labels, int label_dtype, int64_t n, int part,
                                    int parts, const void* slots, int64_t P, int64_t* part_out, void* workspace,
                                    size_t workspace_bytes, dauc_stream_t stream);

int dauc_sort_keys(const float* scores, int64_t n, unsigned* keys_out, void* workspace,
                   size_t workspace_bytes, dauc_stream_t stream);


size_t dauc_bn_workspace_size(int64_t M, int C);
int dauc_bn_act_forward(const void* x, int dtype, int64_t M, int C, const void* residual, int relu,
                        const float* gamma, const float* beta, float* running_mean, float* running_var,
                        float momentum, float eps, void* y, uint8_t* relu_mask, float* save_mean, float* save_invstd,
                        void* workspace, size_t workspace_bytes, dauc_stream_t stream);

int dauc_bn_act_backward(const void* dy, const void* y, const uint8_t* relu_mask, const void* x, int dtype, int64_t M,
                         int C, int relu, const float* gamma, const float* save_mean, const float* save_invstd,
                         void* dres, void* dx, float* dgamma, float* dbeta, void* workspace, size_t workspace_bytes,
                         dauc_stream_t stream);


int dauc_maxpool2d_forward(const void* x, int dtype, int64_t N, int H, int W, int C, int kernel, int stride,
                           int pad, void* y, int8_t* argmax, int Ho, int Wo, dauc_stream_t stream);

int dauc_maxpool2d_backward(const void* dy, const int8_t* argmax, int dtype, int64_t N, int H, int W, int C,
                            int kernel, int stride, int pad, int Ho, int Wo, void* dx, dauc_stream_t stream);


int dauc_slab_sum(const float* part, int64_t S, int64_t n, float* out, dauc_stream_t stream);


size_t dauc_conv3x3_wgrad_workspace_size(int64_t N, int Ho, int Wo, int Ci, int Co);
int dauc_conv3x3_wgrad(const void* x, const void* dy, int dtype, int64_t N, int H, int W, int Ci, int Ho, int Wo,
                       int Co, int stride, float* dw, void* workspace, size_t workspace_bytes, dauc_stream_t stream);


int dauc_conv7x7s2_stem_forward(const void* x, const void* w, int dtype, int64_t N, int H, int W, int Ho, int Wo,
                                void* y, dauc_stream_t stream);
size_t dauc_conv7x7s2_stem_wgrad_workspace_size(int64_t N, int Ho, int Wo);
int dauc_conv7x7s2_stem_wgrad(const void* x, const void* dy, int dtype, int64_t N, int H, int W, int Ho, int Wo,
                              float* dw, void* workspace, size_t workspace_bytes, dauc_stream_t stream);


int dauc_strided_pick(const void* x, int dtype, int64_t N, int H, int W, int C, int stride, void* out,
                      dauc_stream_t stream);
int dauc_strided_add(void* dx, int dtype, int64_t N, int H, int W, int C, int stride, const void* src,
                     dauc_stream_t stream);
int dauc_broadcast_hw(const void* g, int dtype, int64_t N, int64_t HW, int C, void* out, dauc_stream_t stream);

#ifdef __cplusplus
}
#endif

#endif
```

include/dauc_tuning.h:

```cpp
#ifndef DAUC_TUNING_H
#define DAUC_TUNING_H

#include "dauc.h"

#ifdef __cplusplus
extern "C" {
#endif

int dauc_surrogate_fwdbwd_variant(const float* h, int64_t h_stride, const void* y, int y_dtype, int64_t B,
                                  const float* abalpha, const float* p_hat, float* dh, int64_t dh_stride,
                                  double* out64, float* grad3, float* loss, void* workspace,
                                  size_t workspace_bytes, int variant, dauc_stream_t stream);

int dauc_pd_update_dense_variant(float* w, const float* g, const float* w0, float* w_avg, int64_t n,
                                 float lr, float inv_gamma, int variant, dauc_stream_t stream);

int dauc_pair_count_variant(const float* pos, int64_t P, const float* neg, int64_t N,
                            unsigned long long* wins_ties, int variant, dauc_stream_t stream);

int dauc_set_search_mode(int mode);

int dauc_set_direct_fault(int mode);

int dauc_set_index_form(int form);

int dauc_probe_tr16(short* out, dauc_stream_t stream);

int dauc_set_wgrad_form(int form);

#define DAUC_BN_PLAN_WORDS 12
int dauc_bn_launch_plan(int64_t M, int C, int dtype, int64_t out[DAUC_BN_PLAN_WORDS]);

#define DAUC_WGRAD_PLAN_WORDS 18
int dauc_conv3x3_wgrad_launch_plan(int64_t N, int H, int W, int Ci, int Ho, int Wo, int Co, int stride,
                                   int64_t out[DAUC_WGRAD_PLAN_WORDS]);

#ifdef __cplusplus
}
#endif

#endif
```

Baseline: 11180.

## Fuse BN statistic partials into the 1x1 conv forward GEMM epilogue

Adds a HIP 1x1-conv forward kernel that emits per-row-block sum and sum-of-squares partials for the following BatchNorm in its epilogue. A new BN forward entry consumes these partials instead of rereading the conv output to compute statistics. Bottleneck blocks use this path for conv1, the stride-1 downsample and conv3 when fused BN and the GEMM conv are on, with an autotune choice against the library GEMM per shape. It saves one full read of each activation tensor, but the custom GEMM may be slower than the vendor library, and the change adds plan-table and autograd plumbing.

```diff
diff --git a/distributedauc_amd/_lib.py b/distributedauc_amd/_lib.py
--- a/distributedauc_amd/_lib.py
+++ b/distributedauc_amd/_lib.py
@@ -70,6 +70,11 @@
     "dauc_bn_workspace_size": (_sz, [_i64, _int]),
     "dauc_bn_act_forward": (_int, [_vp, _int, _i64, _int, _vp, _int, _vp, _vp, _vp, _vp, _f32, _f32, _vp, _vp, _vp,
                                    _vp, _vp, _sz, _vp]),
+    "dauc_conv1x1_bn_partials_size": (_sz, [_i64, _int, _int]),
+    "dauc_conv1x1_bn_forward": (_int, [_vp, _vp, _int, _i64, _int, _int, _vp, _vp, _sz, ctypes.POINTER(_int),
+                                       ctypes.POINTER(_i64), _vp]),
+    "dauc_bn_act_forward_partials": (_int, [_vp, _int, _i64, _int, _vp, _int, _vp, _vp, _vp, _vp, _f32, _f32, _vp,
+                                            _vp, _vp, _vp, _vp, _int, _i64, _vp, _sz, _vp]),
     "dauc_bn_act_backward": (_int, [_vp, _vp, _vp, _vp, _int, _i64, _int, _int, _vp, _vp, _vp, _vp, _vp, _vp, _vp,
                                     _vp, _sz, _vp]),
     "dauc_maxpool2d_forward": (_int, [_vp, _int, _i64, _int, _int, _int, _int, _int, _int, _vp, _vp, _int, _int,
@@ -100,8 +105,10 @@
     "dauc_set_wgrad_form": (_int, [_int]),
     "dauc_bn_launch_plan": (_int, [_i64, _int, _int, ctypes.POINTER(_i64)]),
     "dauc_conv3x3_wgrad_launch_plan": (_int, [_i64, _int, _int, _int, _int, _int, _int, _int, ctypes.POINTER(_i64)]),
+    "dauc_conv1x1_bn_launch_plan": (_int, [_i64, _int, _int, ctypes.POINTER(_i64)]),
 }
 BN_PLAN_WORDS = 12
+CONV1X1_BN_PLAN_WORDS = 5
 WGRAD_PLAN_WORDS = 18
 TUNING_LIB_PATH = Path(os.environ.get("DAUC_TUNING_LIB", PKG_DIR.parent / "tuning" / "libdauc_tuning.so"))
 
diff --git a/distributedauc_amd/backbone.py b/distributedauc_amd/backbone.py
--- a/distributedauc_amd/backbone.py
+++ b/distributedauc_amd/backbone.py
@@ -13,11 +13,11 @@
 
 
 def _bn_act(fused: bool, bn: nn.BatchNorm2d, x: torch.Tensor, relu: bool = True,
-            residual: torch.Tensor | None = None) -> torch.Tensor:
+            residual: torch.Tensor | None = None, stats=None) -> torch.Tensor:
     if fused and bn.training:
         from .fused_bn import bn_act
 
-        return bn_act(x, bn, relu, residual)
+        return bn_act(x, bn, relu, residual, stats)
     y = bn(x)
     if residual is not None:
         y = y + residual
@@ -241,21 +241,50 @@
         self.downsample = downsample
         self.fused_bn = False
         self.gemm_conv1x1 = False
+        self.conv_bn_stats = True
+        self._cs_cache: dict = {}
+
+    def _bn_stats_candidate(self, x) -> bool:
+        from . import conv1x1 as C
+
+        key = (tuple(x.shape), len(C.plans), len(C._fixed))
+        hit = self._cs_cache.get(key)
+        if hit is None:
+            N, cin, H, W = x.shape
+            s = self.conv2.stride[0]
+            Ho, Wo = (H - 1) // s + 1, (W - 1) // s + 1
+            dt = torch.get_autocast_dtype("cuda") if torch.is_autocast_enabled("cuda") else x.dtype
+            shapes = [(N * H * W, cin, self.conv1.out_channels), (N * Ho * Wo, self.conv3.in_channels,
+                                                                  self.conv3.out_channels)]
+            if self.downsample is not None and self.downsample[0].stride == (1, 1):
+                shapes.append((N * H * W, cin, self.downsample[0].out_channels))
+            hit = self._cs_cache[key] = any(C.fwd_bn_candidate(M, ci, co, dt) for M, ci, co in shapes)
+        return hit
 
     def forward(self, x):
         f, g = self.fused_bn, self.gemm_conv1x1
         down = None if self.downsample is None else self.downsample[0]
-        if g and x.is_cuda:
+        cs = f and g and self.conv_bn_stats and self.training and x.is_cuda and self._bn_stats_candidate(x)
+        st1 = sts = st3 = None
+        if cs:
+            from .conv1x1 import conv1x1, conv1x1_skip
+
+            h, skip, st1, sts = conv1x1_skip(self.conv1, x, down, skip_grad_owned=True, bn_stats=True)
+        elif g and x.is_cuda:
             from .conv1x1 import conv1x1_skip
 
             h, skip = conv1x1_skip(self.conv1, x, down, skip_grad_owned=f and self.training)
         else:
             h, skip = _c1(g, self.conv1, x), (x if down is None else _c1(g, down, x))
         if down is not None:
-            skip = _bn_act(f, self.downsample[1], skip, relu=False)
-        y = _bn_act(f, self.bn1, h)
+            skip = _bn_act(f, self.downsample[1], skip, relu=False, stats=sts)
+        y = _bn_act(f, self.bn1, h, stats=st1)
         y = _bn_act(f, self.bn2, _cw(self.conv2, y))
-        return _bn_act(f, self.bn3, _c1(g, self.conv3, y), residual=skip)
+        if cs:
+            y, st3 = conv1x1(self.conv3, y, bn_stats=True)
+        else:
+            y = _c1(g, self.conv3, y)
+        return _bn_act(f, self.bn3, y, residual=skip, stats=st3)
 
 
 class ResNet(nn.Module):
@@ -329,6 +358,12 @@
                 m.gemm_conv1x1 = bool(enabled)
         return self
 
+    def set_conv_bn_stats(self, enabled: bool = True) -> "ResNet":
+        for m in self.modules():
+            if isinstance(m, Bottleneck):
+                m.conv_bn_stats = bool(enabled)
+        return self
+
     def features(self, x):
         if self.fused_bn and self.training and x.is_cuda and self._counted_bns:
             torch._foreach_add_([m.num_batches_tracked for m in self._counted_bns], 1)
diff --git a/distributedauc_amd/conv1x1.py b/distributedauc_amd/conv1x1.py
--- a/distributedauc_amd/conv1x1.py
+++ b/distributedauc_amd/conv1x1.py
@@ -13,6 +13,7 @@
 __all__ = ["conv1x1", "conv1x1_skip", "Conv1x1Function", "Conv1x1SkipFunction", "plans", "dump_plans"]
 
 plans: dict = {}
+shipped_fwd_bn: dict = {}
 
 _DOWNSAMPLE_BWD = os.environ.get("DAUC_DOWNSAMPLE_BWD", "gemm")
 PLANS_FILE = os.environ.get("DAUC_CONV1X1_PLANS", os.path.join(os.path.dirname(__file__), "conv1x1_plans.json"))
@@ -37,9 +38,10 @@
         doc = json.load(f)
     if doc.get("arch") and torch.cuda.is_available() and doc["arch"] != _arch():
         return
-    for k, eng in doc.get("plans", {}).items():
-        M, cin, cout, dt, direction = k.split(",")
-        plans.setdefault((int(M), int(cin), int(cout), dtypes[dt], direction), eng)
+    for table, into in (("plans", plans), ("plans_fwd_bn", shipped_fwd_bn)):
+        for k, eng in doc.get(table, {}).items():
+            M, cin, cout, dt, direction = k.split(",")
+            into.setdefault((int(M), int(cin), int(cout), dtypes[dt], direction), eng)
 
 
 def dump_plans(path: str) -> None:
@@ -48,7 +50,11 @@
     with open(path, "w") as f:
         json.dump({"device": torch.cuda.get_device_name(0) if torch.cuda.is_available() else None,
                    "arch": _arch() if torch.cuda.is_available() else None,
-                   "plans": {_plan_key(k): v for k, v in sorted(plans.items(), key=lambda kv: _plan_key(kv[0]))}},
+                   "plans": {_plan_key(k): v for k, v in sorted(plans.items(), key=lambda kv: _plan_key(kv[0]))
+                             if k[4] != "fwd_bn"},
+                   "plans_fwd_bn": {_plan_key(k): v for k, v in sorted({**shipped_fwd_bn, **plans}.items(),
+                                                                       key=lambda kv: _plan_key(kv[0]))
+                                    if k[4] == "fwd_bn"}},
                   f, indent=1)
 
 
@@ -143,6 +149,71 @@
     return y, wc
 
 
+def _hip_fwd_bn(x, wc):
+    import ctypes
+
+    N, cin, H, W = x.shape
+    cout = wc.shape[0]
+    M = N * H * W
+    L = _lib.load()
+    nbytes = L.dauc_conv1x1_bn_partials_size(M, cin, cout)
+    if not nbytes or not _cl_ok(x) or not wc.is_contiguous() or wc.data_ptr() % 16:
+        return None
+    y = torch.empty((N, H, W, cout), dtype=x.dtype, device=x.device)
+    partials = torch.empty(nbytes // 4, dtype=torch.float32, device=x.device)
+    nrb, rows = ctypes.c_int(0), ctypes.c_int64(0)
+    rc = L.dauc_conv1x1_bn_forward(_ptr(x), _ptr(wc), _lib.DTYPE_BF16, M, cin, cout, _ptr(y), _ptr(partials), nbytes,
+                                   ctypes.byref(nrb), ctypes.byref(rows), _stream(x.device))
+    if rc == _lib.DAUC_EINVAL:
+        return None
+    check(rc, "dauc_conv1x1_bn_forward")
+    return y.permute(0, 3, 1, 2), (partials, nrb.value, rows.value)
+
+
+def fwd_bn_candidate(M, cin, cout, dtype) -> bool:
+    if _fixed or _FORCE != "auto" or dtype != torch.bfloat16:
+        return False
+    if not _loaded:
+        _load_plans()
+        _loaded.append(True)
+    key = (M, cin, cout, dtype, "fwd_bn")
+    eng = plans.get(key) or shipped_fwd_bn.get(key)
+    if eng is not None:
+        return eng == "hip"
+    return bool(_lib.load().dauc_conv1x1_bn_partials_size(M, cin, cout))
+
+
+def _fwd_bn(x, weight):
+    cout, cin = weight.shape[0], weight.shape[1]
+    M = x.shape[0] * x.shape[2] * x.shape[3]
+    if _fixed or _FORCE != "auto" or x.dtype != torch.bfloat16:
+        return (*_fwd(x, weight), None)
+    key = (M, cin, cout, x.dtype, "fwd_bn")
+    if not _loaded:
+        _load_plans()
+        _loaded.append(True)
+    eng = plans.get(key) or shipped_fwd_bn.get(key)
+    if eng == "lib":
+        return (*_fwd(x, weight), None)
+    wc = _low(weight, x.dtype).reshape(cout, cin)
+    if (not _cl_ok(x) or not wc.is_contiguous() or wc.data_ptr() % 16
+            or not _lib.load().dauc_conv1x1_bn_partials_size(M, cin, cout)):
+        return (*_fwd(x, weight), None)
+    with torch.autocast("cuda", enabled=False):
+        def bn_after(y, stats):
+            from .fused_bn import bn_forward
+
+            bn_forward(y, None, None, None, None, None, 0.0, 1e-5, True, stats)
+
+        if eng is None:
+            eng = _choose(key, {"hip": lambda: bn_after(*_hip_fwd_bn(x, wc)),
+                                "lib": lambda: bn_after(_fwd(x, weight)[0], None)})
+        r = _hip_fwd_bn(x, wc) if eng == "hip" else None
+    if r is not None:
+        return r[0], wc, r[1]
+    return (*_fwd(x, weight), None)
+
+
 def _prep_grad(gy, x, cout):
     N, cin, H, W = x.shape
     gy = gy.to(x.dtype).contiguous(memory_format=torch.channels_last)
@@ -245,30 +316,46 @@
 
 
 class Conv1x1Function(torch.autograd.Function):
+
     @staticmethod
-    def forward(ctx, x, weight):
-        y, wc = _fwd(x, weight)
+    def forward(ctx, x, weight, bn_stats=None):
+        if bn_stats is None:
+            y, wc = _fwd(x, weight)
+        else:
+            y, wc, st = _fwd_bn(x, weight)
         ctx.save_for_backward(x, wc)
         ctx.wdtype = weight.dtype
-        return y
+        if bn_stats is None:
+            return y
+        bn_stats.append(None if st is None else st[1:])
+        if st is None:
+            return y, None
+        ctx.mark_non_differentiable(st[0])
+        return y, st[0]
 
     @staticmethod
-    def backward(ctx, gy):
+    def backward(ctx, gy, *_):
         x, wc = ctx.saved_tensors
         gy, g2 = _prep_grad(gy, x, wc.shape[0])
         dx = _dgrad(gy, g2, x, wc) if ctx.needs_input_grad[0] else None
         dw = _wgrad(gy, g2, x, wc, ctx.wdtype) if ctx.needs_input_grad[1] else None
-        return dx, dw
+        return dx, dw, None
 
 
 class Conv1x1SkipFunction(torch.autograd.Function):
 
     @staticmethod
-    def forward(ctx, x, w1, wd, skip_grad_owned, down_stride=1):
-        y1, wc1 = _fwd(x, w1)
+    def forward(ctx, x, w1, wd, skip_grad_owned, down_stride=1, bn_stats=None):
+        st1 = std = None
+        if bn_stats is None:
+            y1, wc1 = _fwd(x, w1)
+        else:
+            y1, wc1, st1 = _fwd_bn(x, w1)
         ctx.down_stride = int(down_stride)
         if wd is None:
             skip, wcd = x, None
+        elif down_stride == 1 and bn_stats is not None:
+            skip, wcd, std = _fwd_bn(x, wd)
         elif down_stride == 1:
             skip, wcd = _fwd(x, wd)
         else:
@@ -279,10 +366,17 @@
         ctx.save_for_backward(x, wc1, wcd)
         ctx.wdtypes = (w1.dtype, None if wd is None else wd.dtype)
         ctx.skip_grad_owned = bool(skip_grad_owned)
-        return y1, skip
+        if bn_stats is None:
+            return y1, skip
+        parts = []
+        for st in (st1, std):
+            bn_stats.append(None if st is None else st[1:])
+            parts.append(None if st is None else st[0])
+        ctx.mark_non_differentiable(*[p for p in parts if p is not None])
+        return y1, skip, parts[0], parts[1]
 
     @staticmethod
-    def backward(ctx, g1, gs):
+    def backward(ctx, g1, gs, *_):
         x, wc1, wcd = ctx.saved_tensors
         dx = dw1 = dwd = None
         gy1 = g21 = gyd = g2d = None
@@ -331,17 +425,25 @@
                 dwd = dwd_s.to(ctx.wdtypes[1]).view(wcd.shape[0], wcd.shape[1], 1, 1)
             else:
                 dwd = _wgrad(gyd, g2d, xd, wcd, ctx.wdtypes[1])
-        return dx, dw1, dwd, None, None
-
-
-def conv1x1(conv: nn.Conv2d, x: torch.Tensor) -> torch.Tensor:
+        return dx, dw1, dwd, None, None, None
+
+
+def _stats(partials, plan):
+    return None if partials is None or plan is None else (partials, *plan)
+
+
+def conv1x1(conv: nn.Conv2d, x: torch.Tensor, bn_stats: bool = False):
     if (conv.kernel_size != (1, 1) or conv.stride != (1, 1) or conv.groups != 1 or conv.bias is not None
             or conv.padding != (0, 0) or x.device.type != "cuda"
             or not x.is_contiguous(memory_format=torch.channels_last)):
-        return conv(x)
+        return (conv(x), None) if bn_stats else conv(x)
     if torch.is_autocast_enabled("cuda") and x.dtype == torch.float32:
         x = x.to(torch.get_autocast_dtype("cuda"))
-    return Conv1x1Function.apply(x, conv.weight)
+    if not bn_stats:
+        return Conv1x1Function.apply(x, conv.weight)
+    plan: list = []
+    y, partials = Conv1x1Function.apply(x, conv.weight, plan)
+    return y, _stats(partials, plan[0])
 
 
 def _gemm_ok(conv: nn.Conv2d | None, x: torch.Tensor, any_stride: bool = False) -> bool:
@@ -350,11 +452,20 @@
                             and (conv.stride == (1, 1) or (any_stride and conv.stride[0] == conv.stride[1])))
 
 
-def conv1x1_skip(conv: nn.Conv2d, x: torch.Tensor, down: nn.Conv2d | None = None, skip_grad_owned: bool = False):
+def conv1x1_skip(conv: nn.Conv2d, x: torch.Tensor, down: nn.Conv2d | None = None, skip_grad_owned: bool = False,
+                 bn_stats: bool = False):
     if (x.device.type != "cuda" or not x.is_contiguous(memory_format=torch.channels_last)
             or not _gemm_ok(conv, x) or not _gemm_ok(down, x, any_stride=True)):
-        return conv1x1(conv, x), (x if down is None else conv1x1(down, x))
+        if not bn_stats:
+            return conv1x1(conv, x), (x if down is None else conv1x1(down, x))
+        h, st = conv1x1(conv, x, True)
+        skip, sts = (x, None) if down is None else conv1x1(down, x, True)
+        return h, skip, st, sts
     if torch.is_autocast_enabled("cuda") and x.dtype == torch.float32:
         x = x.to(torch.get_autocast_dtype("cuda"))
-    return Conv1x1SkipFunction.apply(x, conv.weight, None if down is None else down.weight, skip_grad_owned,
-                                     1 if down is None else down.stride[0])
+    wd, ds = (None, 1) if down is None else (down.weight, down.stride[0])
+    if not bn_stats:
+        return Conv1x1SkipFunction.apply(x, conv.weight, wd, skip_grad_owned, ds)
+    plan: list = []
+    h, skip, p1, ps = Conv1x1SkipFunction.apply(x, conv.weight, wd, skip_grad_owned, ds, plan)
+    return h, skip, _stats(p1, plan[0]), _stats(ps, plan[1])
diff --git a/distributedauc_amd/csrc/bn_act.hip b/distributedauc_amd/csrc/bn_act.hip
--- a/distributedauc_amd/csrc/bn_act.hip
+++ b/distributedauc_amd/csrc/bn_act.hip
@@ -14,7 +14,6 @@
 
 constexpr int kBnThreads = 256;
 constexpr int kDefaultPartThreads = 512;
-constexpr int kMaxRowBlocks = 2048;
 constexpr int kFinThreads = 1024;
 constexpr int kFinSubsets = kFinThreads / 16;
 
@@ -522,18 +521,13 @@
 }
 
 template <typename T>
-int bn_forward_t(const T* x, int64_t M, int C, const T* res, int relu, const float* gamma, const float* beta,
-                 float* running_mean, float* running_var, float momentum, float eps, T* y, unsigned char* mask,
-                 float* save_mean, float* save_invstd, void* ws, size_t ws_bytes, hipStream_t st) {
-    Geometry g;
-    const int th = kDefaultPartThreads;
-    if (make_geometry(M, C, sizeof(T), g, th) != DAUC_OK) return DAUC_EINVAL;
-    if (ws == nullptr || ws_bytes < ws_bytes_for(C) || !aligned16p(ws)) return DAUC_EINVAL;
-    if ((running_mean == nullptr) != (running_var == nullptr)) return DAUC_EINVAL;
-    const BnWs w = carve(ws, C);
-    launch_partial<T, true, false>(th, g, x, nullptr, nullptr, nullptr, M, C, nullptr, w.partials, st);
-    hipLaunchKernelGGL(bn_fwd_finalize_kernel, dim3((C + 63) / 64), dim3(kFinThreads), 0, st, w.partials, g.nrb,
-                       g.rows, M, C, gamma, beta, running_mean, running_var, momentum, eps, save_mean, save_invstd, w.c0, w.c1, w.c3);
+int bn_forward_tail(const T* x, int64_t M, int C, const T* res, int relu, const float* gamma, const float* beta,
+                    float* running_mean, float* running_var, float momentum, float eps, T* y, unsigned char* mask,
+                    float* save_mean, float* save_invstd, const float* partials, int nrb, int64_t rows,
+                    const BnWs& w, hipStream_t st) {
+    hipLaunchKernelGGL(bn_fwd_finalize_kernel, dim3((C + 63) / 64), dim3(kFinThreads), 0, st, partials, nrb, rows, M,
+                       C, gamma, beta, running_mean, running_var, momentum, eps, save_mean, save_invstd, w.c0, w.c1,
+                       w.c3);
     int rc = launch_status();
     if (rc != DAUC_OK) return rc;
     if (relu && mask && res)
@@ -547,6 +541,28 @@
     if (relu) return launch_elementwise<T, false, 0, true, false>(x, nullptr, nullptr, y, M, C, w.c0, w.c1, nullptr, w.c3, st);
     if (res) return launch_elementwise<T, false, 0, false, true>(x, nullptr, res, y, M, C, w.c0, w.c1, nullptr, w.c3, st);
     return launch_elementwise<T, false, 0, false, false>(x, nullptr, nullptr, y, M, C, w.c0, w.c1, nullptr, w.c3, st);
+}
+
+template <typename T>
+int bn_forward_t(const T* x, int64_t M, int C, const T* res, int relu, const float* gamma, const float* beta,
+                 float* running_mean, float* running_var, float momentum, float eps, T* y, unsigned char* mask,
+                 float* save_mean, float* save_invstd, const float* partials, int nrb, int64_t rows, void* ws,
+                 size_t ws_bytes, hipStream_t st) {
+    Geometry g;
+    const int th = kDefaultPartThreads;
+    if (make_geometry(M, C, sizeof(T), g, th) != DAUC_OK) return DAUC_EINVAL;
+    if (ws == nullptr || ws_bytes < ws_bytes_for(C) || !aligned16p(ws)) return DAUC_EINVAL;
+    if ((running_mean == nullptr) != (running_var == nullptr)) return DAUC_EINVAL;
+    const BnWs w = carve(ws, C);
+    if (partials != nullptr) {
+        if (nrb < 1 || nrb > kMaxRowBlocks || rows < 1 || !aligned16p(partials)) return DAUC_EINVAL;
+        if (int64_t(nrb - 1) * rows >= M || (M - int64_t(nrb - 1) * rows) > rows) return DAUC_EINVAL;
+        return bn_forward_tail(x, M, C, res, relu, gamma, beta, running_mean, running_var, momentum, eps, y, mask,
+                               save_mean, save_invstd, partials, nrb, rows, w, st);
+    }
+    launch_partial<T, true, false>(th, g, x, nullptr, nullptr, nullptr, M, C, nullptr, w.partials, st);
+    return bn_forward_tail(x, M, C, res, relu, gamma, beta, running_mean, running_var, momentum, eps, y, mask,
+                           save_mean, save_invstd, w.partials, g.nrb, g.rows, w, st);
 }
 
 template <typename T>
@@ -596,10 +612,11 @@
     return C > 0 ? ws_bytes_for(C) : 0;
 }
 
-int dauc_bn_act_forward(const void* x, int dtype, int64_t M, int C, const void* residual, int relu,
-                        const float* gamma, const float* beta, float* running_mean, float* running_var,
-                        float momentum, float eps, void* y, uint8_t* relu_mask, float* save_mean, float* save_invstd,
-                        void* workspace, size_t workspace_bytes, dauc_stream_t stream) {
+static int bn_act_forward_any(const void* x, int dtype, int64_t M, int C, const void* residual, int relu,
+                              const float* gamma, const float* beta, float* running_mean, float* running_var,
+                              float momentum, float eps, void* y, uint8_t* relu_mask, float* save_mean,
+                              float* save_invstd, const float* partials, int nrb, int64_t rows, void* workspace,
+                              size_t workspace_bytes, dauc_stream_t stream) {
     if (x == nullptr || y == nullptr || save_mean == nullptr || save_invstd == nullptr) return DAUC_EINVAL;
     if (!all_aligned({x, residual, y})) return DAUC_EINVAL;
     if (relu_mask != nullptr && !relu) return DAUC_EINVAL;
@@ -607,13 +624,32 @@
     if (dtype == DAUC_DTYPE_BF16)
         return bn_forward_t(static_cast<const __hip_bfloat16*>(x), M, C, static_cast<const __hip_bfloat16*>(residual),
                             relu, gamma, beta, running_mean, running_var, momentum, eps,
-                            static_cast<__hip_bfloat16*>(y), relu_mask, save_mean, save_invstd, workspace,
-                            workspace_bytes, st);
+                            static_cast<__hip_bfloat16*>(y), relu_mask, save_mean, save_invstd, partials, nrb, rows,
+                            workspace, workspace_bytes, st);
     if (dtype == DAUC_DTYPE_F32)
         return bn_forward_t(static_cast<const float*>(x), M, C, static_cast<const float*>(residual), relu, gamma,
                             beta, running_mean, running_var, momentum, eps, static_cast<float*>(y), relu_mask,
-                            save_mean, save_invstd, workspace, workspace_bytes, st);
+                            save_mean, save_invstd, partials, nrb, rows, workspace, workspace_bytes, st);
     return DAUC_EINVAL;
+}
+
+int dauc_bn_act_forward(const void* x, int dtype, int64_t M, int C, const void* residual, int relu,
+                        const float* gamma, const float* beta, float* running_mean, float* running_var,
+                        float momentum, float eps, void* y, uint8_t* relu_mask, float* save_mean, float* save_invstd,
+                        void* workspace, size_t workspace_bytes, dauc_stream_t stream) {
+    return bn_act_forward_any(x, dtype, M, C, residual, relu, gamma, beta, running_mean, running_var, momentum, eps, y,
+                              relu_mask, save_mean, save_invstd, nullptr, 0, 0, workspace, workspace_bytes, stream);
+}
+
+int dauc_bn_act_forward_partials(const void* x, int dtype, int64_t M, int C, const void* residual, int relu,
+                                 const float* gamma, const float* beta, float* running_mean, float* running_var,
+                                 float momentum, float eps, void* y, uint8_t* relu_mask, float* save_mean,
+                                 float* save_invstd, const float* partials, int nrb, int64_t rows, void* workspace,
+                                 size_t workspace_bytes, dauc_stream_t stream) {
+    if (partials == nullptr) return DAUC_EINVAL;
+    return bn_act_forward_any(x, dtype, M, C, residual, relu, gamma, beta, running_mean, running_var, momentum, eps, y,
+                              relu_mask, save_mean, save_invstd, partials, nrb, rows, workspace, workspace_bytes,
+                              stream);
 }
 
 int dauc_bn_act_backward(const void* dy, const void* y, const uint8_t* relu_mask, const void* x, int dtype, int64_t M,
diff --git a/distributedauc_amd/csrc/conv1x1_bn.hip b/distributedauc_amd/csrc/conv1x1_bn.hip
--- /dev/null
+++ b/distributedauc_amd/csrc/conv1x1_bn.hip
@@ -0,0 +1,249 @@
+
+#include <hip/hip_bf16.h>
+
+#include "dauc_internal.h"
+#ifdef DAUC_TUNING
+#include "dauc_tuning.h"
+#endif
+
+namespace dauc {
+namespace {
+
+typedef __bf16 bf16x4 __attribute__((ext_vector_type(4)));
+typedef __bf16 bf16x8 __attribute__((ext_vector_type(8)));
+typedef float f32x4v __attribute__((ext_vector_type(4)));
+typedef unsigned u32x4 __attribute__((ext_vector_type(4)));
+
+constexpr int kThreads = 256;
+constexpr int kGridTarget = 512;
+static_assert(kGridTarget <= kMaxRowBlocks, "one partial row block per workgroup");
+
+__device__ __forceinline__ void cvt8(const u32x4& u, float (&v)[8]) {
+#pragma unroll
+    for (int i = 0; i < 4; ++i) {
+        v[2 * i] = __uint_as_float(u[i] << 16);
+        v[2 * i + 1] = __uint_as_float(u[i] & 0xffff0000u);
+    }
+}
+
+template <int CIN, int COUT, int TM>
+struct Tile {
+    static constexpr int KS = CIN / 32;
+    static constexpr int CT = COUT / 64;
+    static constexpr int XC = CIN / 8;
+    static constexpr int XV = TM * XC / kThreads;
+    static constexpr int XROW = CIN + 8;
+    static constexpr int OROW = COUT + 8;
+    static constexpr int TPR = COUT / 8;
+    static constexpr int RPB = kThreads / TPR;
+    static constexpr int U = TM / RPB;
+    static constexpr int XS = TM * XROW, OS = TM * OROW;
+    static_assert(CIN % 32 == 0 && COUT % 64 == 0 && TM % 16 == 0, "MFMA tiling");
+    static_assert((TM * XC) % kThreads == 0 && XV >= 1, "x staging");
+    static_assert(TPR <= 64 && kThreads % TPR == 0 && TM % RPB == 0 && U >= 1, "store loop");
+    static_assert((XS + OS) * 2 >= 2 * kThreads * 8 * 4, "the final reduction reuses the tiles");
+    static_assert((XS + OS) * 2 <= 80 * 1024, "two workgroups per CU");
+};
+
+template <typename G>
+__device__ __forceinline__ void load_x(u32x4 (&st)[G::XV], const unsigned short* __restrict__ xt, int count,
+                                       int cin) {
+#pragma unroll
+    for (int u = 0; u < G::XV; ++u) {
+        const int q = threadIdx.x + kThreads * u, p = q / G::XC, v = q % G::XC;
+        st[u] = *reinterpret_cast<const u32x4*>(xt + (int64_t(p < count ? p : 0) * cin + 8 * v));
+    }
+}
+
+template <int CIN, int COUT, int TM>
+__global__ __launch_bounds__(kThreads) __attribute__((amdgpu_waves_per_eu(2, 2))) void conv1x1_bn_kernel(
+    const unsigned short* __restrict__ x, const unsigned short* __restrict__ w, int64_t M, int64_t rows,
+    unsigned short* __restrict__ y, float* __restrict__ partials) {
+    using G = Tile<CIN, COUT, TM>;
+    __shared__ __attribute__((aligned(16))) short smem[G::XS + G::OS];
+    short* xs = smem;
+    short* os = smem + G::XS;
+    const int tid = threadIdx.x, lane = tid & 63, wave = tid >> 6;
+    const int grp = lane >> 4, col = lane & 15;
+    const int cobase = wave * (COUT / 4);
+    const int64_t rs = int64_t(blockIdx.x) * rows;
+    const int64_t re = rs + rows < M ? rs + rows : M;
+
+    bf16x8 wa[G::CT][G::KS];
+#pragma unroll
+    for (int ct = 0; ct < G::CT; ++ct)
+#pragma unroll
+        for (int s = 0; s < G::KS; ++s)
+            wa[ct][s] = __builtin_bit_cast(
+                bf16x8, *reinterpret_cast<const u32x4*>(w + ((cobase + 16 * ct + col) * CIN + 32 * s + 8 * grp)));
+
+    const int cv = tid % G::TPR, r0 = tid / G::TPR;
+    float k[8], s1[8], s2[8];
+#pragma unroll
+    for (int i = 0; i < 8; ++i) k[i] = s1[i] = s2[i] = 0.f;
+
+    u32x4 st[G::XV];
+    {
+        const int64_t left = re - rs;
+        load_x<G>(st, x + rs * CIN, left < TM ? int(left) : TM, CIN);
+    }
+    for (int64_t t = rs; t < re; t += TM) {
+        const int count = re - t < TM ? int(re - t) : TM;
+        __syncthreads();
+#pragma unroll
+        for (int u = 0; u < G::XV; ++u) {
+            const int q = tid + kThreads * u, p = q / G::XC, v = q % G::XC;
+            *reinterpret_cast<u32x4*>(xs + (p * G::XROW + 8 * v)) = st[u];
+        }
+        __syncthreads();
+        if (t + TM < re) {
+            const int64_t left = re - (t + TM);
+            load_x<G>(st, x + (t + TM) * CIN, left < TM ? int(left) : TM, CIN);
+        }
+        for (int pt = 0; pt < TM / 16; ++pt) {
+            if (16 * pt >= count) break;
+            const int px = 16 * pt + col;
+            f32x4v acc[G::CT];
+#pragma unroll
+            for (int ct = 0; ct < G::CT; ++ct) acc[ct] = f32x4v{0.f, 0.f, 0.f, 0.f};
+#pragma unroll
+            for (int s = 0; s < G::KS; ++s) {
+                const bf16x8 b = __builtin_bit_cast(
+                    bf16x8, *reinterpret_cast<const u32x4*>(xs + (px * G::XROW + 32 * s + 8 * grp)));
+#pragma unroll
+                for (int ct = 0; ct < G::CT; ++ct)
+                    acc[ct] = __builtin_amdgcn_mfma_f32_16x16x32_bf16(wa[ct][s], b, acc[ct], 0, 0, 0);
+            }
+#pragma unroll
+            for (int ct = 0; ct < G::CT; ++ct)
+                *reinterpret_cast<bf16x4*>(os + (px * G::OROW + cobase + 16 * ct + 4 * grp)) =
+                    __builtin_convertvector(acc[ct], bf16x4);
+        }
+        __syncthreads();
+        if (t == rs) cvt8(*reinterpret_cast<const u32x4*>(os + 8 * cv), k);
+        unsigned short* yt = y + t * COUT;
+#pragma unroll
+        for (int u = 0; u < G::U; ++u) {
+            const int p = r0 + G::RPB * u;
+            if (p < count) {
+                const u32x4 vv = *reinterpret_cast<const u32x4*>(os + (p * G::OROW + 8 * cv));
+                *reinterpret_cast<u32x4*>(yt + (int64_t(p) * COUT + 8 * cv)) = vv;
+                float f[8];
+                cvt8(vv, f);
+#pragma unroll
+                for (int i = 0; i < 8; ++i) {
+                    const float d = f[i] - k[i];
+                    s1[i] += d;
+                    s2[i] += d * d;
+                }
+            }
+        }
+    }
+
+    __syncthreads();
+    float* r1 = reinterpret_cast<float*>(smem);
+    float* r2 = r1 + kThreads * 8;
+#pragma unroll
+    for (int i = 0; i < 8; ++i) {
+        r1[r0 * COUT + 8 * cv + i] = s1[i];
+        r2[r0 * COUT + 8 * cv + i] = s2[i];
+    }
+    __syncthreads();
+    float* prow = partials + int64_t(blockIdx.x) * 3 * COUT;
+    for (int j = tid; j < 2 * COUT; j += kThreads) {
+        const int stat = j / COUT, c = j % COUT;
+        const float* src = stat ? r2 : r1;
+        float acc = 0.f;
+        for (int q = 0; q < G::RPB; ++q) acc += src[q * COUT + c];
+        prow[stat * COUT + c] = acc;
+    }
+    if (r0 == 0) {
+#pragma unroll
+        for (int i = 0; i < 8; ++i) prow[2 * COUT + 8 * cv + i] = k[i];
+    }
+}
+
+int row_tile(int cin, int cout) {
+    if (cin == 64 && cout == 64) return 128;
+    if ((cin == 64 && cout == 256) || (cin == 256 && cout == 64) || (cin == 256 && cout == 128)) return 64;
+    if ((cin == 128 && cout == 512) || (cin == 512 && cout == 128)) return 32;
+    return 0;
+}
+
+struct ConvBnPlan {
+    int tm;
+    int64_t tpw;
+    int nrb;
+    int64_t rows;
+};
+
+int make_plan(int64_t M, int cin, int cout, ConvBnPlan& p) {
+    p.tm = row_tile(cin, cout);
+    if (p.tm == 0 || M <= 0 || M > (int64_t(1) << 40)) return DAUC_EINVAL;
+    const int64_t tiles = (M + p.tm - 1) / p.tm;
+    p.tpw = (tiles + kGridTarget - 1) / kGridTarget;
+    p.rows = p.tpw * p.tm;
+    p.nrb = static_cast<int>((M + p.rows - 1) / p.rows);
+    return DAUC_OK;
+}
+
+template <int CIN, int COUT, int TM>
+void launch(const ConvBnPlan& p, const void* x, const void* w, int64_t M, void* y, float* partials, hipStream_t st) {
+    hipLaunchKernelGGL((conv1x1_bn_kernel<CIN, COUT, TM>), dim3(p.nrb), dim3(kThreads), 0, st,
+                       static_cast<const unsigned short*>(x), static_cast<const unsigned short*>(w), M, p.rows,
+                       static_cast<unsigned short*>(y), partials);
+}
+
+}
+}
+
+using namespace dauc;
+
+extern "C" {
+
+size_t dauc_conv1x1_bn_partials_size(int64_t M, int Cin, int Cout) {
+    ConvBnPlan p;
+    if (make_plan(M, Cin, Cout, p) != DAUC_OK) return 0;
+    return size_t(p.nrb) * 3 * size_t(Cout) * sizeof(float);
+}
+
+int dauc_conv1x1_bn_forward(const void* x, const void* w, int dtype, int64_t M, int Cin, int Cout, void* y,
+                            float* partials, size_t partials_bytes, int* nrb, int64_t* rows,
+                            dauc_stream_t stream) {
+    if (x == nullptr || w == nullptr || y == nullptr || partials == nullptr || nrb == nullptr || rows == nullptr)
+        return DAUC_EINVAL;
+    if (dtype != DAUC_DTYPE_BF16) return DAUC_EINVAL;
+    if ((reinterpret_cast<uintptr_t>(x) | reinterpret_cast<uintptr_t>(w) | reinterpret_cast<uintptr_t>(y) |
+         reinterpret_cast<uintptr_t>(partials)) & 15u)
+        return DAUC_EINVAL;
+    ConvBnPlan p;
+    if (make_plan(M, Cin, Cout, p) != DAUC_OK) return DAUC_EINVAL;
+    if (partials_bytes < size_t(p.nrb) * 3 * size_t(Cout) * sizeof(float)) return DAUC_EINVAL;
+    hipStream_t st = as_hip(stream);
+    if (Cin == 64 && Cout == 64) launch<64, 64, 128>(p, x, w, M, y, partials, st);
+    else if (Cin == 64 && Cout == 256) launch<64, 256, 64>(p, x, w, M, y, partials, st);
+    else if (Cin == 256 && Cout == 64) launch<256, 64, 64>(p, x, w, M, y, partials, st);
+    else if (Cin == 256 && Cout == 128) launch<256, 128, 64>(p, x, w, M, y, partials, st);
+    else if (Cin == 128 && Cout == 512) launch<128, 512, 32>(p, x, w, M, y, partials, st);
+    else launch<512, 128, 32>(p, x, w, M, y, partials, st);
+    *nrb = p.nrb;
+    *rows = p.rows;
+    return launch_status();
+}
+
+#ifdef DAUC_TUNING
+int dauc_conv1x1_bn_launch_plan(int64_t M, int Cin, int Cout, int64_t out[DAUC_CONV1X1_BN_PLAN_WORDS]) {
+    if (out == nullptr) return DAUC_EINVAL;
+    ConvBnPlan p;
+    const int rc = make_plan(M, Cin, Cout, p);
+    if (rc != DAUC_OK) return rc;
+    out[0] = p.tm;
+    out[1] = p.tpw;
+    out[2] = p.nrb;
+    out[3] = p.rows;
+    out[4] = (M % p.rows) != 0 ? 1 : 0;
+    return DAUC_OK;
+}
+#endif
+
+}
diff --git a/distributedauc_amd/csrc/dauc_internal.h b/distributedauc_amd/csrc/dauc_internal.h
--- a/distributedauc_amd/csrc/dauc_internal.h
+++ b/distributedauc_amd/csrc/dauc_internal.h
@@ -8,6 +8,8 @@
 namespace dauc {
 
 constexpr int kWave = 64;
+
+constexpr int kMaxRowBlocks = 2048;
 
 typedef float f32x4 __attribute__((ext_vector_type(4)));
 
diff --git a/distributedauc_amd/fused_bn.py b/distributedauc_amd/fused_bn.py
--- a/distributedauc_amd/fused_bn.py
+++ b/distributedauc_amd/fused_bn.py
@@ -6,7 +6,7 @@
 from . import _lib
 from .ops import _ptr, _stream, check, workspaces
 
-__all__ = ["supported", "bn_act", "BnActFunction"]
+__all__ = ["supported", "bn_act", "bn_forward", "BnActFunction"]
 
 _DTYPES = {torch.float32: 1, torch.bfloat16: 2}
 
@@ -25,27 +25,41 @@
     return 256 % tpr == 0 and cv % tpr == 0
 
 
+def bn_forward(x, weight, bias, residual, running_mean, running_var, momentum, eps, relu, stats=None):
+    N, C, H, W = x.shape
+    M = N * H * W
+    dev = x.device
+    L = _lib.load()
+    y = torch.empty_like(x, memory_format=torch.channels_last)
+    mask = torch.empty(M * C * x.element_size() // 16, dtype=torch.uint8, device=dev) if relu else None
+    mean = torch.empty(C, dtype=torch.float32, device=dev)
+    invstd = torch.empty(C, dtype=torch.float32, device=dev)
+    ws = workspaces.get(dev, "bn", L.dauc_bn_workspace_size(M, C))
+    if residual is not None:
+        if residual.shape != x.shape or residual.dtype != x.dtype:
+            raise ValueError("residual must match x in shape and dtype")
+        residual = residual.contiguous(memory_format=torch.channels_last)
+    head = (_ptr(x), _DTYPES[x.dtype], M, C, _ptr(residual), int(relu), _ptr(weight), _ptr(bias),
+            _ptr(running_mean), _ptr(running_var), float(momentum), float(eps), _ptr(y), _ptr(mask), _ptr(mean),
+            _ptr(invstd))
+    if stats is None:
+        check(L.dauc_bn_act_forward(*head, _ptr(ws), ws.numel(), _stream(dev)), "dauc_bn_act_forward")
+    else:
+        partials, nrb, rows = stats
+        if partials.dtype != torch.float32 or partials.numel() < nrb * 3 * C:
+            raise ValueError("partials must hold nrb x 3 x C fp32 words")
+        check(L.dauc_bn_act_forward_partials(*head, _ptr(partials), int(nrb), int(rows), _ptr(ws), ws.numel(),
+                                             _stream(dev)), "dauc_bn_act_forward_partials")
+    return y, mask, mean, invstd
+
+
 class BnActFunction(torch.autograd.Function):
 
     @staticmethod
-    def forward(ctx, x, weight, bias, residual, running_mean, running_var, momentum, eps, relu):
-        N, C, H, W = x.shape
-        M = N * H * W
-        dev = x.device
-        L = _lib.load()
-        y = torch.empty_like(x, memory_format=torch.channels_last)
-        mask = torch.empty(M * C * x.element_size() // 16, dtype=torch.uint8, device=dev) if relu else None
-        mean = torch.empty(C, dtype=torch.float32, device=dev)
-        invstd = torch.empty(C, dtype=torch.float32, device=dev)
-        ws = workspaces.get(dev, "bn", L.dauc_bn_workspace_size(M, C))
-        if residual is not None:
-            if residual.shape != x.shape or residual.dtype != x.dtype:
-                raise ValueError("residual must match x in shape and dtype")
-            residual = residual.contiguous(memory_format=torch.channels_last)
-        check(L.dauc_bn_act_forward(_ptr(x), _DTYPES[x.dtype], M, C, _ptr(residual), int(relu), _ptr(weight),
-                                    _ptr(bias), _ptr(running_mean), _ptr(running_var), float(momentum), float(eps),
-                                    _ptr(y), _ptr(mask), _ptr(mean), _ptr(invstd), _ptr(ws), ws.numel(), _stream(dev)),
-              "dauc_bn_act_forward")
+    def forward(ctx, x, weight, bias, residual, running_mean, running_var, momentum, eps, relu, partials=None,
+                nrb=0, rows=0):
+        y, mask, mean, invstd = bn_forward(x, weight, bias, residual, running_mean, running_var, momentum, eps, relu,
+                                           None if partials is None else (partials, nrb, rows))
         ctx.save_for_backward(x, mask, weight, mean, invstd)
         ctx.relu = bool(relu)
         ctx.has_residual = residual is not None
@@ -71,11 +85,11 @@
                                      _ptr(weight), _ptr(mean), _ptr(invstd), _ptr(dres), _ptr(dx), _ptr(dgamma),
                                      _ptr(dbeta), _ptr(ws), ws.numel(), _stream(dev)),
               "dauc_bn_act_backward")
-        return dx, dgamma, dbeta, dres, None, None, None, None, None
+        return dx, dgamma, dbeta, dres, None, None, None, None, None, None, None, None
 
 
 def bn_act(x: torch.Tensor, bn: nn.BatchNorm2d, relu: bool = True,
-           residual: torch.Tensor | None = None) -> torch.Tensor:
+           residual: torch.Tensor | None = None, stats=None) -> torch.Tensor:
     if x.device.type != "cuda":
         raise RuntimeError("fused BN runs on the GPU only (libdauc.so); no CPU path")
     if not supported(x):
@@ -87,4 +101,6 @@
         bn.num_batches_tracked.add_(1)
         if bn.momentum is None:
             momentum = 1.0 / float(bn.num_batches_tracked.item())
-    return BnActFunction.apply(x, bn.weight, bn.bias, residual, rm, rv, momentum, bn.eps, relu)
+    if stats is None:
+        return BnActFunction.apply(x, bn.weight, bn.bias, residual, rm, rv, momentum, bn.eps, relu)
+    return BnActFunction.apply(x, bn.weight, bn.bias, residual, rm, rv, momentum, bn.eps, relu, *stats)
diff --git a/include/dauc.h b/include/dauc.h
--- a/include/dauc.h
+++ b/include/dauc.h
@@ -135,6 +135,17 @@
                         float momentum, float eps, void* y, uint8_t* relu_mask, float* save_mean, float* save_invstd,
                         void* workspace, size_t workspace_bytes, dauc_stream_t stream);
 
+size_t dauc_conv1x1_bn_partials_size(int64_t M, int Cin, int Cout);
+int dauc_conv1x1_bn_forward(const void* x, const void* w, int dtype, int64_t M, int Cin, int Cout, void* y,
+                            float* partials, size_t partials_bytes, int* nrb, int64_t* rows,
+                            dauc_stream_t stream);
+
+int dauc_bn_act_forward_partials(const void* x, int dtype, int64_t M, int C, const void* residual, int relu,
+                                 const float* gamma, const float* beta, float* running_mean, float* running_var,
+                                 float momentum, float eps, void* y, uint8_t* relu_mask, float* save_mean,
+                                 float* save_invstd, const float* partials, int nrb, int64_t rows, void* workspace,
+                                 size_t workspace_bytes, dauc_stream_t stream);
+
 int dauc_bn_act_backward(const void* dy, const void* y, const uint8_t* relu_mask, const void* x, int dtype, int64_t M,
                          int C, int relu, const float* gamma, const float* save_mean, const float* save_invstd,
                          void* dres, void* dx, float* dgamma, float* dbeta, void* workspace, size_t workspace_bytes,
diff --git a/include/dauc_tuning.h b/include/dauc_tuning.h
--- a/include/dauc_tuning.h
+++ b/include/dauc_tuning.h
@@ -35,6 +35,9 @@
 int dauc_conv3x3_wgrad_launch_plan(int64_t N, int H, int W, int Ci, int Ho, int Wo, int Co, int stride,
                                    int64_t out[DAUC_WGRAD_PLAN_WORDS]);
 
+#define DAUC_CONV1X1_BN_PLAN_WORDS 5
+int dauc_conv1x1_bn_launch_plan(int64_t M, int Cin, int Cout, int64_t out[DAUC_CONV1X1_BN_PLAN_WORDS]);
+
 #ifdef __cplusplus
 }
 #endif
```

Result: no change. 11200 (median of 3 runs) (+0.1%).
